# beer-asr/beer

Hardware: AMD Instinct MI355X
Metric: frames/sec per VB iteration (E+M) (higher is better)
Workload: dtype f32

## Files before the change

beer_amd/_hip.py:

```python

import ctypes
import os
import threading

import torch

_HERE = os.path.dirname(os.path.abspath(__file__))
LIB_PATH = os.environ.get('BEER_HIP_LIB') or os.path.join(_HERE, 'csrc', 'libbeer_hip.so')

F32, F64, I16 = 0, 1, 2
FULL, DIAG, ISO = 0, 1, 2
SEG = 8
MAX_HUBS = 4
COV_CODE = {'full': FULL, 'diagonal': DIAG, 'isotropic': ISO}
EINVAL = -100000


class HipUnavailable(RuntimeError):
    'Raised when the HIP extension or the GPU is missing (no CPU fallback).'


class HipError(RuntimeError):
    rc = None


class HipInvalid(HipError):
    rc = EINVAL


_lib = None


def lib():
    global _lib
    if _lib is None:
        if not os.path.exists(LIB_PATH):
            raise HipUnavailable(
                f'{LIB_PATH} is missing: build it with `python -m beer_amd.build` '
                '(beer_amd has no CPU fallback)')
        _lib = ctypes.CDLL(LIB_PATH)
        _declare(_lib)
        _options_from_env(_lib)
    return _lib


OPTIONS = {'ax_max_frames': (0, 'BEER_AX_MAXFRAMES'), 'accf_rounds': (1, 'BEER_ACCF_ROUNDS'),
           'accfi_waves': (2, 'BEER_ACCFI_WAVES'), 'lnfi': (3, 'BEER_LNFI'),
           'fb_log': (4, 'BEER_FB_LOG'), 'k1_lds': (5, 'BEER_K1_LDS')}


def _options_from_env(l):
    for name, (code, env) in OPTIONS.items():
        text = os.environ.get(env)
        if text is None:
            continue
        try:
            value = int(text)
        except ValueError:
            raise ValueError(f'{env}={text!r}: expected an integer') from None
        if l.beer_hip_set_option(code, value) != 0:
            raise ValueError(f'{env}={value}: outside the range of option {name!r} '
                             '(include/beer_hip.h)')


def set_option(name, value):
    code = OPTIONS[name][0]
    old = lib().beer_hip_get_option(code)
    if lib().beer_hip_set_option(code, int(value)) != 0:
        raise ValueError(f'option {name!r}: value {value} out of range')
    return old


def get_option(name):
    return lib().beer_hip_get_option(OPTIONS[name][0])


c_p, c_i, c_l, c_d = ctypes.c_void_p, ctypes.c_int, ctypes.c_int64, ctypes.c_double
c_z = ctypes.c_size_t


class Graph(ctypes.Structure):
    _fields_ = [('n_states', ctypes.c_int32), ('n_arcs', ctypes.c_int32),
                ('n_in_seg', ctypes.c_int32), ('n_out_seg', ctypes.c_int32),
                ('init', c_p), ('final', c_p),
                ('in_ptr', c_p), ('in_src', c_p), ('in_dst', c_p), ('in_w', c_p),
                ('in_seg', c_p), ('in_row_seg', c_p),
                ('out_ptr', c_p), ('out_dst', c_p), ('out_src', c_p), ('out_w', c_p),
                ('out_seg', c_p), ('out_row_seg', c_p), ('lowdeg', c_p)]


class GraphLowDeg(ctypes.Structure):
    _fields_ = [('n_arcs', ctypes.c_int32), ('n_hubs', ctypes.c_int32),
                ('in_ptr', c_p), ('in_src', c_p), ('in_w', c_p),
                ('out_ptr', c_p), ('out_dst', c_p), ('out_w', c_p),
                ('hub_src_id', c_p), ('hub_src_w', c_p), ('hub_dst_id', c_p),
                ('hub_dst_w', c_p), ('src_ptr', c_p), ('src_list', c_p),
                ('dst_ptr', c_p), ('dst_list', c_p)]


class Batch(ctypes.Structure):
    _fields_ = [('nutt', ctypes.c_int32), ('max_states', ctypes.c_int32),
                ('max_arcs', ctypes.c_int32), ('max_segs', ctypes.c_int32),
                ('all_lowdeg', ctypes.c_int32), ('n_graphs', ctypes.c_int32),
                ('frame_off', c_p), ('llh_off', c_p), ('graph_id', c_p),
                ('graphs', c_p), ('pdf_off', c_p), ('pdf_ids', c_p),
                ('max_degree', ctypes.c_int32), ('max_hubs', ctypes.c_int32),
                ('max_hub_members', ctypes.c_int32), ('reserved', ctypes.c_int32),
                ('order', c_p)]


class CatMap(ctypes.Structure):
    _fields_ = [('arc_cat', c_p), ('last_cat', c_p), ('arc_off', c_p), ('state_off', c_p)]


class Bigram(ctypes.Structure):
    _fields_ = [('n_states', ctypes.c_int32), ('n_phones', ctypes.c_int32),
                ('max_degree', ctypes.c_int32), ('reserved', ctypes.c_int32),
                ('init', c_p), ('final', c_p),
                ('in_ptr', c_p), ('in_src', c_p), ('in_w', c_p),
                ('out_ptr', c_p), ('out_dst', c_p), ('out_w', c_p),
                ('src', c_p), ('dst', c_p), ('block_w', c_p),
                ('src_slot', c_p), ('dst_slot', c_p), ('pdf_ids', c_p)]


FB_WAVE, FB_LOWDEG, FB_GENERAL, FB_GENERAL_BIG = 0x1000, 0x2000, 0x3000, 0x4000


def fb_family(route):
    return route & 0xF000


SAMPLE_ARCS_LDS, SAMPLE_QUAD = 0x100, 0x200


def sample_chunk(route):
    return route & 0xFF


def sample_waves(route):
    return (route >> 12) & 0xF


ESTEP_PLAIN, ESTEP_PACKED, ESTEP_IMAGE = 0, 1, 2
ARG_PC_LLH, ARG_LOG_NORM, ARG_RESPS, ARG_LLH_SUM, ARG_LABELS, ARG_SCALED, ARG_LOG_WEIGHTS = \
    1, 2, 4, 8, 16, 32, 64
ESTEP_GENERIC, ESTEP_EXACT_F32, ESTEP_EXACT_F64, ESTEP_LLHX, ESTEP_LNFI = \
    0x10000000, 0x20000000, 0x30000000, 0x40000000, 0x50000000
ESTEP_GENERIC_PASS1, ESTEP_GENERIC_FUSED, ESTEP_GENERIC_NORMALISE, ESTEP_GENERIC_LABELS = 1, 2, 3, 4
ESTEP_X_PACKED, ESTEP_X_LNO, ESTEP_X_IMG, ESTEP_X_BL = 0x100, 0x200, 0x400, 0x800
ESTEP_X_NARROW, ESTEP_X_LANE_MAJOR, ESTEP_X_PADDED, ESTEP_X_XT = 0x1000, 0x2000, 0x4000, 0x8000


def estep_family(route):
    return route & 0x70000000


def estep_route(entry, dtype_code_, cov, D, S, G, args, workspace_bytes):
    return lib().beer_estep_route(entry, dtype_code_, cov, D, S, G, args, workspace_bytes)


ACC_PLAIN, ACC_PACKED, ACC_FUSED = 0, 1, 2
ARG_STATE_RESPS, ARG_IMAGE = 128, 256
ACC_GENERIC, ACC_EXACT_F32, ACC_EXACT_F64, ACC_DIAG, ACC_ACCX, ACC_ACCF = \
    0x10000000, 0x20000000, 0x30000000, 0x40000000, 0x50000000, 0x60000000
ACC_SR = 0x100
ACC_D_PARTIAL = 0x200
ACC_X_SX, ACC_X_XT_REUSED = 0x200, 0x400
ACC_F_BLK, ACC_F_IMAGE = 0x200, 0x400


def accumulate_family(route):
    return route & 0x70000000


def accumulate_route(entry, dtype_code_, cov, T, D, S, G, args, workspace_bytes):
    return lib().beer_accumulate_route(entry, dtype_code_, cov, T, D, S, G, args, workspace_bytes)


DENSE_LLH, DENSE_BACKWARD, DENSE_ACCUMULATE = 0, 1, 2
DENSE_PLAIN, DENSE_GEMM3 = 0x10000000, 0x20000000
DENSE_T64x128, DENSE_T128x64, DENSE_T128x128 = 1, 2, 3
DENSE_AK, DENSE_BK = 0x10, 0x20


def dense_family(route):
    return route & 0x70000000


def dense_chain(route):
    return (route >> 8 & 0xFF) * 32


def dense_route(op, dtype_code_, T, Q, K):
    return lib().beer_dense_route(op, dtype_code_, T, Q, K)


SGRAD_GENERIC, SGRAD_FULL, SGRAD_DIAG, SGRAD_CHUNKED = 0x10000000, 0x20000000, 0x30000000, 0x40000000


def sgrad_family(route):
    return route & 0x70000000


def sgrad_form(route):
    return route & 0x0FFFFFFF


def frames_llh_backward_route(dtype_code_, cov, T, D, K, workspace_bytes):
    return lib().beer_frames_llh_backward_route(dtype_code_, cov, T, D, K, workspace_bytes)


BIGRAM_MAX_PHONES = 128
BIGRAM_MAX_STATES = 512


class FeaConf(ctypes.Structure):
    _fields_ = [('flen', ctypes.c_int32), ('fstep', ctypes.c_int32),
                ('fft_len', ctypes.c_int32), ('mode', ctypes.c_int32),
                ('nfilters', ctypes.c_int32), ('apply_log', ctypes.c_int32),
                ('n_dct', ctypes.c_int32), ('add_energy', ctypes.c_int32),
                ('preemph', ctypes.c_double), ('log_offset', ctypes.c_double),
                ('norm', ctypes.c_double),
                ('window', c_p), ('filters', c_p), ('filt_lo', c_p), ('filt_hi', c_p),
                ('dct', c_p), ('lifter', c_p)]


_four = [c_i, c_i, c_i, c_p, c_p, c_p, c_p, c_p, c_p]
_from = [c_i, c_i, c_i, c_p, c_p, c_p, c_p, c_p, c_p]
_dir = [c_i, c_i, c_i, c_p, c_p, c_p]
_gam = [c_i, c_i, c_p, c_p, c_p, c_p]
SIGNATURES = {
    'beer_hip_version': [],
    'beer_hip_device_count': [],
    'beer_hip_set_option': [c_i, c_i],
    'beer_hip_get_option': [c_i],
    'beer_mixtureset_packed_supported': [c_i, c_i, c_i, c_i],
    'beer_nw_expected_stats': _four, 'beer_nw_log_norm': _four, 'beer_nw_natural': _four,
    'beer_nw_from_natural': _from,
    'beer_nw_expected_stats_log_norm': [c_i, c_i, c_i, c_p, c_p, c_p, c_p, c_p, c_p, c_p],
    'beer_nw_update': [c_i, c_i, c_i, c_p, c_p, c_p, c_p, c_p, c_p, c_p, c_p, c_p],
    'beer_ng_expected_stats': _four, 'beer_ng_log_norm': _four, 'beer_ng_natural': _four,
    'beer_ng_from_natural': _from,
    'beer_ing_expected_stats': _four, 'beer_ing_log_norm': _four, 'beer_ing_natural': _four,
    'beer_ing_from_natural': _from,
    'beer_dirichlet_expected_stats': _dir, 'beer_dirichlet_log_norm': _dir,
    'beer_dirichlet_natural': _dir, 'beer_dirichlet_from_natural': _dir,
    'beer_dirichlet_log_weights': _dir,
    'beer_sb_transform_stats': [c_i, c_i, c_p, c_p, c_p, c_p],
    'beer_sb_log_weights': [c_i, c_i, c_p, c_p, c_p, c_p, c_p],
    'beer_sb_set_log_weights': [c_i, c_i, c_i, c_p, c_p, c_p, c_p],
    'beer_sb_set_transform_stats': [c_i, c_i, c_i, c_p, c_p, c_p, c_p],
    'beer_gamma_expected_stats': _gam, 'beer_gamma_log_norm': _gam,
    'beer_gamma_natural': _gam,
    'beer_gamma_from_natural': [c_i, c_i, c_p, c_p, c_p, c_p],
    'beer_kl_div': [c_i, c_i, c_i, c_p, c_p, c_p, c_p, c_p, c_p, c_p],
    'beer_natural_grad_step': [c_i, c_l, c_p, c_p, c_p, c_d, c_p, c_p],
    'beer_suffstats_expand': [c_i, c_i, c_l, c_i, c_p, c_p, c_p],
    'beer_mixtureset_estep': [c_i, c_i, c_l, c_i, c_i, c_i, c_p, c_p, c_p, c_p, c_d,
                              c_p, c_p, c_p, c_p, c_p, c_z, c_p],
    'beer_normal_accumulate': [c_i, c_i, c_l, c_i, c_i, c_i, c_p, c_p, c_p, c_p, c_p, c_z,
                               c_p],
    'beer_mixture_estep_packed': [c_i, c_l, c_i, c_i, c_p, c_p, c_p, c_p, c_p, c_p, c_p, c_z,
                                  c_p],
    'beer_normal_accumulate_packed': [c_i, c_l, c_i, c_i, c_p, c_p, c_p, c_p, c_z, c_p],
    'beer_mixtureset_estep_packed': [c_i, c_l, c_i, c_i, c_i, c_p, c_p, c_p, c_p, c_p, c_p, c_p,
                                     c_z, c_p],
    'beer_mixtureset_accumulate_packed': [c_i, c_l, c_i, c_i, c_i, c_p, c_p, c_p, c_p, c_p, c_z,
                                          c_p],
    'beer_unpack_resps': [c_l, c_i, c_p, c_p, c_p],
    'beer_mixtureset_accumulate_fused': [c_i, c_l, c_i, c_i, c_i, c_p, c_p, c_p, c_p, c_p, c_p,
                                         c_p, c_p, c_z, c_p],
    'beer_frame_image': [c_i, c_l, c_i, c_p, c_p, c_z, c_p],
    'beer_mixtureset_lognorm_image': [c_i, c_l, c_i, c_i, c_i, c_p, c_p, c_p, c_p, c_p, c_p, c_p,
                                      c_z, c_p],
    'beer_estep_route': [c_i, c_i, c_i, c_i, c_i, c_i, ctypes.c_uint, c_z],
    'beer_accumulate_route': [c_i, c_i, c_i, c_l, c_i, c_i, c_i, ctypes.c_uint, c_z],
    'beer_dense_route': [c_i, c_i, c_l, c_i, c_i],
    'beer_frames_llh_backward_route': [c_i, c_i, c_l, c_i, c_i, c_z],
    'beer_pack_resps': [c_l, c_i, c_i, c_i, c_p, c_p, c_p, c_p, c_p],
    'beer_weights_from_acc': [c_i, c_i, c_i, c_p, c_p, c_p],
    'beer_tied_lognorm': [c_i, c_l, c_i, c_i, c_p, c_p, c_p, c_p, c_p, c_p],
    'beer_tied_accumulate': [c_i, c_l, c_i, c_i, c_p, c_p, c_p, c_p, c_p, c_p, c_p, c_p],
    'beer_hmm_gather': [c_i, c_p, c_i, c_p, c_d, c_p, c_p],
    'beer_hmm_forward_backward': [c_i, c_p, c_p, c_p, c_p, c_p, c_p, c_p, c_p, c_p, c_p],
    'beer_hmm_posteriors_fused': [c_i, c_p, c_i, c_p, c_d, c_p, c_p, c_p, c_i, c_p, c_p, c_p,
                                  c_p, c_p],
    'beer_hmm_posteriors_fused_counts': [c_i, c_p, c_i, c_p, c_d, c_p, c_p, c_p, c_i, c_p, c_p,
                                         c_p, c_p, c_p, c_p, c_p],
    'beer_hmm_forward_backward_counts': [c_i, c_p, c_p, c_p, c_p, c_p, c_p, c_p, c_p, c_p, c_p,
                                         c_p],
    'beer_hmm_last_frame_sum': [c_i, c_p, c_p, c_p, c_p],
    'beer_hmm_refresh_weights': [c_i, c_l, c_p, c_p, c_p, c_p, c_p],
    'beer_hmm_posteriors_fused_cat': [c_i, c_p, c_i, c_p, c_d, c_p, c_p, c_p, c_i, c_p, c_p, c_p,
                                      c_p, c_p, c_p],
    'beer_hmm_forward_backward_cat': [c_i, c_p, c_p, c_p, c_p, c_p, c_p, c_p, c_p, c_p, c_p],
    'beer_hmm_path_counts_cat': [c_p, c_p, c_p, c_p, c_p],
    'beer_hmm_fb_log_count': [c_p, c_p, c_p, c_p],
    'beer_hmm_fb_route': [c_i, c_p, c_i, c_i],
    'beer_hmm_posteriors_bigram': [c_i, c_p, ctypes.c_int32, c_l, c_p, c_p, c_i, c_p, c_d, c_p,
                                   c_p, c_p, c_i, c_p, c_p],
    'beer_hmm_bigram_route': [c_i, c_p, ctypes.c_int32, ctypes.c_int32],
    'beer_hmm_viterbi': [c_i, c_p, c_p, c_p, c_p, c_i, c_p],
    'beer_hmm_sample_paths': [c_i, c_p, c_p, c_p, ctypes.c_int32, c_p, c_p, c_i, c_p],
    'beer_hmm_sample_route': [c_i, c_p, ctypes.c_int32],
    'beer_hmm_trans_posteriors': [c_i, c_l, c_i, c_p, c_p, c_p, c_p, c_p, c_p],
    'beer_hmm_path_posteriors': [c_i, c_p, c_p, c_p, c_p, c_p, c_p],
    'beer_hmm_scatter': [c_i, c_p, c_i, c_p, c_p, c_d, c_p, c_p, c_p, c_p],
    'beer_segment_sum': [c_i, ctypes.c_int32, c_p, c_p, c_p, c_p],
    'beer_dense_llh': [c_i, c_l, c_i, c_i, c_p, c_p, c_d, c_p, c_p],
    'beer_dense_llh_backward': [c_i, c_l, c_i, c_i, c_p, c_p, c_p, c_p, c_p],
    'beer_dense_accumulate': [c_i, c_l, c_i, c_i, c_i, c_p, c_p, c_p, c_p, c_p],
    'beer_rowdot': [c_i, c_l, c_i, c_p, c_p, c_p, c_p],
    'beer_softmax_groups': [c_i, c_l, c_i, c_i, c_p, c_p, c_p, c_p, c_p],
    'beer_features_signal_mean': [c_i, ctypes.c_int32, c_p, c_p, c_p, c_p],
    'beer_features_extract': [c_i, ctypes.c_int32, c_p, c_p, c_l, c_p, c_p, c_p, c_p,
                              ctypes.c_int32, c_p],
    'beer_features_deltas': [ctypes.c_int32, c_p, c_l, ctypes.c_int32, ctypes.c_int32,
                             ctypes.c_int32, c_p, c_p, c_p],
    'beer_features_cmn': [ctypes.c_int32, c_p, ctypes.c_int32, ctypes.c_int32, c_p, c_p],
    'beer_copy_pinned': [c_p, c_p, c_z, c_p],
    'beer_clock_probe': [c_p, c_i, c_p],
    'beer_suffstats_mean': [c_i, c_i, c_l, c_i, c_i, c_p, c_p, c_p],
    'beer_suffstats_backward': [c_i, c_i, c_l, c_i, c_i, c_p, c_p, c_p, c_p],
    'beer_frames_llh_backward': [c_i, c_i, c_l, c_i, c_i, c_p, c_p, c_p, c_p, c_p, c_p, c_z, c_p],
}


c_pp = ctypes.POINTER(ctypes.c_void_p)
HOST_SIGNATURES = {
    'beer_graph_compile': [ctypes.c_int32, c_p, c_l, c_p, c_p, c_p, ctypes.c_int32,
                           ctypes.c_int32, c_pp],
    'beer_aligraphs_compile': [ctypes.c_int32, c_p, c_p, c_p, c_p, c_p, c_p, c_p, c_p, c_l,
                               c_p, c_p, c_pp],
    'beer_graphset_from_csr': [c_l, c_p, c_p, c_p, c_p, c_p, c_p, c_p, c_p, c_pp],
    'beer_graphset_free': [c_p],
    'beer_graphset_sizes': [c_p, c_p, c_p, c_p],
    'beer_graphset_export': [c_p, c_p, c_p, c_p, c_p, c_p, c_p],
    'beer_graphset_image_bytes': [c_p, c_i, c_p],
    'beer_graphset_image': [c_p, c_i, c_p, ctypes.c_uint64, c_p],
}

SIZE_QUERIES = {
    'beer_estep_workspace_bytes': [c_i, c_i, c_i, c_i, c_i],
    'beer_accumulate_workspace_bytes': [c_i, c_i, c_i, c_i, c_i],
    'beer_accumulate_frames_workspace_bytes': [c_i, c_i, c_l, c_i, c_i, c_i],
    'beer_packed_resps_bytes': [c_l, c_i, c_i],
    'beer_accumulate_fused_workspace_bytes': [c_i, c_i, c_i, c_i],
    'beer_frame_image_bytes': [c_i, c_l, c_i],
    'beer_accumulate_packed_workspace_bytes': [c_i, c_l, c_i, c_i],
    'beer_mixtureset_accumulate_packed_workspace_bytes': [c_i, c_l, c_i, c_i, c_i],
    'beer_hmm_fb_scratch_doubles': [c_i, c_p, c_i],
    'beer_frames_llh_backward_workspace_bytes': [c_i, c_i, c_l, c_i, c_i],
}


def _declare(l):
    for name, args in SIGNATURES.items():
        fn = getattr(l, name)
        fn.argtypes = args
        fn.restype = c_i
    for name, args in HOST_SIGNATURES.items():
        fn = getattr(l, name)
        fn.argtypes = args
        fn.restype = c_i
    for name, args in SIZE_QUERIES.items():
        fn = getattr(l, name)
        fn.argtypes = args
        fn.restype = c_z


def dtype_code(dtype, exact=False):
    if dtype == torch.float32:
        return F32 | EXACT if exact else F32
    if dtype == torch.float64:
        return F64
    raise TypeError(f'beer_amd kernels take float32 or float64 tensors, got {dtype}')


def require_device():
    if not torch.cuda.is_available():
        raise HipUnavailable('beer_amd needs an AMD GPU (gfx950); there is no CPU fallback')
    lib()
    return torch.device('cuda', torch.cuda.current_device())


def on_device(t, dtype=None):
    dev = require_device()
    if t.device.type != 'cuda':
        t = t.to(dev)
    if dtype is not None and t.dtype != dtype:
        t = t.to(dtype)
    return t.contiguous()


def ptr(t):
    return None if t is None else ctypes.c_void_p(t.data_ptr())


def stream_id():
    return torch.cuda.current_stream().cuda_stream


def stream():
    return ctypes.c_void_p(stream_id())


def call(name, *args):
    rc = getattr(lib(), name)(*args, stream())
    if rc == EINVAL:
        raise HipInvalid(f'{name} failed: invalid argument')
    if rc != 0:
        err = HipError(f'{name} failed: hipError {-rc}')
        err.rc = rc
        raise err


EXACT = 0x10
F32_MODES = ('exact', 'bf16x3')
_f32_mode = ['exact' if os.environ.get('BEER_F32_MODE') in ('exact', 'f32') else 'bf16x3']


def set_f32_mode(mode):
    if mode not in F32_MODES:
        raise ValueError(f'f32 mode {mode!r}: expected one of {F32_MODES}')
    _f32_mode[0] = mode


def get_f32_mode():
    return _f32_mode[0]


FAST_MIN_FRAMES = 16384
MAX_DIM_F32 = 96
MAX_DIM_FAST = 128


def f32_fast_ok(X):
    return X.dtype == torch.float32 and get_f32_mode() == 'bf16x3' and \
        X.shape[0] >= FAST_MIN_FRAMES and X.shape[1] <= MAX_DIM_FAST


class exact_f32:

    def __enter__(self):
        self.old = get_f32_mode()
        set_f32_mode('exact')

    def __exit__(self, *exc):
        set_f32_mode(self.old)


def call_host(name, *args):
    rc = getattr(lib(), name)(*args)
    if rc != 0:
        raise HipInvalid(f'{name} failed: invalid argument')


_workspaces = {}


def scratch(key, nbytes, device):
    if nbytes == 0:
        return None, 0
    key = (key, device, stream_id())
    buf = _workspaces.get(key)
    if buf is None or buf.numel() < nbytes:
        buf = _workspaces[key] = torch.empty(nbytes, dtype=torch.uint8, device=device)
    return buf, nbytes


def workspace(query, dtype, cov, D, S, G, device):
    return scratch((query, dtype, cov, D, S, G),
                   getattr(lib(), query)(dtype_code(dtype), cov, D, S, G), device)


def frames_workspace(dtype, exact, cov, T, D, S, G, device):
    return scratch(('frames', dtype, cov, D, S, G), lib().beer_accumulate_frames_workspace_bytes(
        dtype_code(dtype, exact), cov, T, D, S, G), device)


def packed_workspace(cov, T, D, K, device, sets=None):
    if sets is None:
        nbytes = lib().beer_accumulate_packed_workspace_bytes(cov, T, D, K)
    else:
        nbytes = lib().beer_mixtureset_accumulate_packed_workspace_bytes(cov, T, D, *sets)
    return scratch(('packed', cov, D, K), nbytes, device)


_staging = threading.local()


def _staging_buffer(nbytes):
    ring = _staging.__dict__.setdefault('ring', [])
    if not ring:
        for _ in range(4):
            ring.append([torch.empty(1 << 20, dtype=torch.uint8, pin_memory=True),
                         torch.cuda.Event()])
    nxt = _staging.__dict__.get('next', 0)
    slot = ring[nxt % len(ring)]
    _staging.next = nxt + 1
    slot[1].synchronize()
    if slot[0].numel() < nbytes:
        slot[0] = torch.empty(max(nbytes, 2 * slot[0].numel()), dtype=torch.uint8,
                              pin_memory=True)
# ... 38 lines not shown
```

beer_amd/csrc/estep.hip:

```cpp

#include "common.h"
#include "estep_mfma.h"

using namespace beer;

namespace {

constexpr int kFrameTile = 64;
constexpr int kLlhThreads = 256;
constexpr int kCompChunk = 64;

template <typename T, int COV>
__global__ __launch_bounds__(kLlhThreads) void llh_kernel(
    int64_t nframes, int D, int K, const T* __restrict__ X, const T* __restrict__ expT,
    const T* __restrict__ logw, double stat_scale, T* __restrict__ pc_llh,
    T* __restrict__ w_out, int fuse_G, T* __restrict__ log_norm,
    double* __restrict__ llh_sum) {
    extern __shared__ __attribute__((aligned(16))) char smem[];
    const int ldx = D + 1;
    T* xs = reinterpret_cast<T*>(smem);
    T* outs = xs + kFrameTile * ldx;
    const int ldo = kCompChunk + 1;
    const int Q = stats_dim(COV, D);
    const int64_t t0 = (int64_t)blockIdx.x * kFrameTile;
// ... 275 lines not shown
                         ws_bytes >= beer_mfma::estep_workspace_bytes(elem, cov, D, S, G);
    const bool split_ws = elem == 4 && !exact &&
                          ws_bytes >= beer_mfma::estepx_workspace_bytes(cov, D, S, G) &&
                          beer_mfma::estepx_workspace_bytes(cov, D, S, G) > 0;
    const bool aligned_x = split_ws && beer_mfma::supported_llh_x(D, S, G);
    const bool padded = split_ws && !comp_resps && beer_mfma::supported_llh_split(D, S, G);
    p.use_x = aligned_x || padded;
    const bool mfma_ok = !labels && !pc_llh && unscaled && ws && (aligned || p.use_x) &&
                         (log_norm || comp_resps || llh_sum);
    p.use_x = mfma_ok && p.use_x;
    p.exact_mfma = mfma_ok && !p.use_x;
    if (p.need_norm && !comp_resps && !mfma_ok && !(G == 1 && log_norm)) return p;
    if (labels && !(pc_llh || comp_resps)) return p;
    p.pc_in_resps = labels && !pc_llh;
    p.fuse = !mfma_ok && p.need_norm && !labels && (kCompChunk % G == 0) && (comp_resps || G == 1);
    p.rc = BEER_OK;
    return p;
}

template <typename T>
int estep_launch(int cov, int64_t nframes, int D, int S, int G, const void* X, const void* expT,
                 const void* logw, const int64_t* labels, double stat_scale, void* pc_llh,
                 void* log_norm, void* comp_resps, double* llh_sum, void* ws, size_t ws_bytes,
                 void* stream, bool exact) {
    BEER_REQUIRE(nframes >= 0 && X && expT);
    const EstepPlan p = estep_plan(sizeof(T), exact, cov, D, S, G, pc_llh, log_norm, comp_resps,
                                   llh_sum, labels, stat_scale == 1.0, ws, ws_bytes);
    if (p.rc != BEER_OK || nframes == 0) return p.rc;
    hipStream_t s = as_stream(stream);
    if (p.use_x)
        return beer_mfma::estep_bf16x3(cov, nframes, D, S, G, (const float*)X, (const float*)expT,
                                       (const float*)logw, (float*)comp_resps, (float*)log_norm,
                                       llh_sum, ws, ws_bytes, s);
    if (p.exact_mfma)
        return sizeof(T) == 4
                   ? beer_mfma::estep_f32(cov, nframes, D, S, G, (const float*)X,
                                          (const float*)expT, (const float*)logw,
                                          (float*)comp_resps, (float*)log_norm, llh_sum, ws,
                                          ws_bytes, s)
                   : beer_mfma::estep_f64(cov, nframes, D, S, G, (const double*)X,
                                          (const double*)expT, (const double*)logw,
                                          (double*)comp_resps, (double*)log_norm, llh_sum, ws,
                                          ws_bytes, s);
    const int K = S * G;
    void* pc = p.pc_in_resps ? comp_resps : pc_llh;
    static_assert(BEER_FULL == 0 && BEER_DIAG == 1 && BEER_ISO == 2, "pass1 is indexed by cov");
    constexpr decltype(&llh_launch<T, BEER_FULL>) pass1[] = {
        llh_launch<T, BEER_FULL>, llh_launch<T, BEER_DIAG>, llh_launch<T, BEER_ISO>};
    const int rc = pass1[cov](nframes, D, K, X, expT, logw, stat_scale, pc,
                              p.need_norm ? comp_resps : nullptr, p.fuse ? G : 0,
                              p.fuse ? log_norm : nullptr, p.fuse ? llh_sum : nullptr, s);
    if (rc != BEER_OK) return rc;
    if (labels) {
        hipLaunchKernelGGL(labels_kernel<T>, dim3((unsigned)((nframes + 255) / 256)), dim3(256), 0,
                           s, nframes, K, labels, (const T*)pc, (T*)comp_resps, (T*)log_norm,
                           llh_sum);
        BEER_LAUNCH_CHECK();
    } else if (p.need_norm && !p.fuse) {
        const int64_t n = nframes * S;
        hipLaunchKernelGGL(normalise_kernel<T>, dim3((unsigned)((n + 255) / 256)), dim3(256), 0, s,
                           nframes, S, G, (T*)comp_resps, (T*)log_norm, true, llh_sum);
        BEER_LAUNCH_CHECK();
    }
    return BEER_OK;
}

template <typename T, int COV>
int acc_launch(int64_t nframes, int D, int S, int G, const void* X, const void* cr,
               const void* sr, double* acc, hipStream_t s) {
    const int K = S * G, Q = stats_dim(COV, D);
    const int gx = (Q + kAccThreads - 1) / kAccThreads, gy = (K + kAccKB - 1) / kAccKB;
    int64_t gz = (256LL * 4 + (int64_t)gx * gy - 1) / ((int64_t)gx * gy);
    const int64_t min_frames = nframes >= 65536 ? 512 : kAccTile;
    const int64_t max_z = (nframes + min_frames - 1) / min_frames;
    if (gz > max_z) gz = max_z;
    if (gz < 1) gz = 1;
    if (gz > 65535) gz = 65535;
    const beer_mfma::FrameSplit z = beer_mfma::frame_split(nframes, gz, kAccTile);
    const size_t lds = ((size_t)kAccTile * D + (size_t)kAccTile * kAccKB) * sizeof(T);
    hipLaunchKernelGGL((accumulate_kernel<T, COV>), dim3(gx, gy, (unsigned)z.gz), dim3(kAccThreads),
                       lds, s, nframes, D, S, G, (const T*)X, (const T*)cr, (const T*)sr, z.fpb, acc);
    BEER_LAUNCH_CHECK();
    return BEER_OK;
}

struct AccPlan {
    int rc;
    bool diag;
    bool exact_mfma;
};

AccPlan accumulate_plan(size_t elem, bool exact, int cov, int64_t nframes, int D, int S, int G,
                        bool cr, bool sr, bool ws, size_t ws_bytes) {
    AccPlan p = {};
    p.rc = BEER_EINVAL;
    if (!(nframes >= 0 && D >= 1 && S >= 1 && G >= 1 && cov >= 0 && cov <= 2)) return p;
    p.rc = BEER_OK;
    p.diag = elem == 4 && !exact && cr && !sr &&
             beer_mfma::supported_acc_diag(cov, nframes, D, S * G);
    p.exact_mfma = !p.diag && cr && ws && beer_mfma::supported_acc(D, S * G, elem) &&
                   ws_bytes >= beer_mfma::acc_workspace_bytes(cov, D, S * G, elem);
    return p;
}

template <typename T>
int accumulate_launch(int cov, int64_t nframes, int D, int S, int G, const void* X,
                      const void* cr, const void* sr, double* acc, void* ws, size_t ws_bytes,
                      void* stream, bool exact) {
    const AccPlan p = accumulate_plan(sizeof(T), exact, cov, nframes, D, S, G, cr, sr, ws, ws_bytes);
    BEER_REQUIRE(p.rc == BEER_OK && X && acc);
    if (nframes == 0) return BEER_OK;
    hipStream_t s = as_stream(stream);
    if (p.diag)
        return beer_mfma::acc_diag_bf16x3(cov, nframes, D, S * G, (const float*)X,
                                          (const float*)cr, acc, ws, ws_bytes, s);
    if (p.exact_mfma)
        return sizeof(T) == 4
                   ? beer_mfma::acc_f32(cov, nframes, D, S, G, (const float*)X, (const float*)cr,
                                        (const float*)sr, acc, ws, ws_bytes, s)
                   : beer_mfma::acc_f64(cov, nframes, D, S, G, (const double*)X,
                                        (const double*)cr, (const double*)sr, acc, ws, ws_bytes,
                                        s);
    constexpr decltype(&acc_launch<T, BEER_FULL>) generic[] = {
        acc_launch<T, BEER_FULL>, acc_launch<T, BEER_DIAG>, acc_launch<T, BEER_ISO>};
    return generic[cov](nframes, D, S, G, X, cr, sr, acc, s);
}

template <typename T>
int segment_sum_launch(int32_t nutt, const int64_t* frame_off, const void* v, double* out,
                       void* stream) {
    BEER_REQUIRE(nutt >= 0);
    if (nutt == 0) return BEER_OK;
    hipLaunchKernelGGL(segment_sum_kernel<T>, dim3(nutt), dim3(256), 0, as_stream(stream),
                       frame_off, (const T*)v, out);
    BEER_LAUNCH_CHECK();
    return BEER_OK;
}

int estepx_refusal(int entry, bool set, int cov, int D, int S, int G, unsigned args,
                   size_t ws_bytes) {
    const bool packed = entry == BEER_ESTEP_PACKED, resps = args & BEER_ARG_RESPS;
    BEER_REQUIRE(D >= 1 && S >= 1 && G >= 1 && cov >= 0 && cov <= 2);
    BEER_REQUIRE(!(args & (BEER_ARG_PC_LLH | BEER_ARG_LABELS | BEER_ARG_SCALED)));
    if (packed)
        BEER_REQUIRE(resps && (set ? beer_mixtureset_packed_supported(cov, D, S, G)
                                   : S == 1 && (args & BEER_ARG_LOG_WEIGHTS)));
    else
        BEER_REQUIRE((args & BEER_ARG_LOG_NORM) && !resps);
    return beer_mfma::llhx_form(cov, D, S, G, packed, packed, !packed, ws_bytes).rc;
}

int estepx_entry(int entry, bool set, int cov, int64_t T, int D, int S, int G, const float* X,
                 const float* exp_stats, const float* logw, const void* image, float* log_norm,
                 void* resps, double* llh_sum, void* ws, size_t ws_bytes, void* stream) {
    const unsigned args = (log_norm ? BEER_ARG_LOG_NORM : 0u) | (resps ? BEER_ARG_RESPS : 0u) |
                          (llh_sum ? BEER_ARG_LLH_SUM : 0u) | (logw ? BEER_ARG_LOG_WEIGHTS : 0u);
    const int rc = estepx_refusal(entry, set, cov, D, S, G, args, ws ? ws_bytes : 0);
    if (rc != BEER_OK || T == 0) return rc;
    return beer_mfma::estep_bf16x3(cov, T, D, S, G, X, exp_stats, logw, (float*)resps, log_norm,
                                   llh_sum, ws, ws_bytes, as_stream(stream),
                                   entry == BEER_ESTEP_PACKED, image);
}

int accx_refusal(bool set, int cov, int64_t T, int D, int S, int G, size_t ws_bytes) {
    BEER_REQUIRE(T >= 0 && D >= 1 && S >= 1 && G >= 1 && cov >= 0 && cov <= 2);
    BEER_REQUIRE(!set || beer_mixtureset_packed_supported(cov, D, S, G));
    BEER_REQUIRE(beer_mfma::accx_form(cov, D, S * G, S, G, set).rc == BEER_OK);
    const size_t need = beer_mfma::accx_layout(cov, T, D, S * G, S, G, set).bytes;
    BEER_REQUIRE(need > 0 && ws_bytes >= need);
    return BEER_OK;
}
int accf_refusal(int cov, int64_t T, int D, int S, int G, size_t ws_bytes) {
    BEER_REQUIRE(T >= 0 && D >= 1 && S >= 1 && G >= 1 && cov >= 0 && cov <= 2);
    BEER_REQUIRE(beer_mfma::accf_form(cov, D, S, G, false).rc == BEER_OK);
    const size_t need = beer_mfma::accf_layout(cov, D, S, G).bytes;
    BEER_REQUIRE(need > 0 && ws_bytes >= need);
    return BEER_OK;
}

}

extern "C" {

int beer_mixtureset_estep(int dtype, int cov, int64_t T, int D, int S, int G, const void* X,
                          const void* exp_stats, const void* log_weights,
                          const int64_t* labels, double stat_scale, void* pc_llh,
                          void* log_norm, void* comp_resps, double* llh_sum, void* workspace,
                          size_t workspace_bytes, void* stream) {
    const bool exact = (dtype & BEER_EXACT) != 0;
    BEER_DISPATCH(dtype & ~BEER_EXACT, estep_launch, cov, T, D, S, G, X, exp_stats, log_weights,
                  labels, stat_scale, pc_llh, log_norm, comp_resps, llh_sum, workspace,
                  workspace_bytes, stream, exact);
}

int beer_estep_route(int entry, int dtype, int cov, int D, int S, int G, unsigned args,
                     size_t workspace_bytes) {
    const bool exact = (dtype & BEER_EXACT) != 0;
    dtype &= ~BEER_EXACT;
    BEER_REQUIRE(dtype == BEER_F32 || dtype == BEER_F64);
    const bool resps = args & BEER_ARG_RESPS, labels = args & BEER_ARG_LABELS;
    bool packed = false;
    if (entry == BEER_ESTEP_PLAIN) {
        const EstepPlan p = estep_plan(dtype == BEER_F64 ? 8 : 4, exact, cov, D, S, G,
                                       args & BEER_ARG_PC_LLH, args & BEER_ARG_LOG_NORM, resps,
                                       args & BEER_ARG_LLH_SUM, labels, !(args & BEER_ARG_SCALED),
                                       workspace_bytes > 0, workspace_bytes);
        if (p.rc != BEER_OK) return p.rc;
        if (p.exact_mfma) {
            const beer_mfma::LlhForm f = beer_mfma::llh_form(S, G);
            return (dtype == BEER_F64 ? BEER_ESTEP_EXACT_F64 : BEER_ESTEP_EXACT_F32) | f.NT |
                   f.GQ << 5 | f.jw << 8 | (f.nchunks > 0xfff ? 0xfff : f.nchunks) << 16;
        }
        if (!p.use_x)
            return BEER_ESTEP_GENERIC | (labels ? BEER_ESTEP_GENERIC_LABELS
                                         : !p.need_norm ? BEER_ESTEP_GENERIC_PASS1
                                         : p.fuse ? BEER_ESTEP_GENERIC_FUSED
                                                  : BEER_ESTEP_GENERIC_NORMALISE);
    } else if (entry == BEER_ESTEP_PACKED || entry == BEER_ESTEP_IMAGE) {
        BEER_REQUIRE(dtype == BEER_F32 && !exact);
        BEER_REQUIRE(estepx_refusal(entry, S != 1, cov, D, S, G, args, workspace_bytes) == BEER_OK);
        packed = entry == BEER_ESTEP_PACKED;
    } else {
        return BEER_EINVAL;
    }
    const beer_mfma::LlhxForm x = beer_mfma::llhx_form(cov, D, S, G, resps, packed,
                                                       entry == BEER_ESTEP_IMAGE, workspace_bytes);
    if (x.rc != BEER_OK) return x.rc;
    const int nchunks = (x.nchunks > 0xfff ? 0xfff : x.nchunks) << 16;
    if (x.lnfi) return BEER_ESTEP_LNFI | x.NT | x.nku << 5 | x.lnfi_g << 8 | nchunks;
    return BEER_ESTEP_LLHX | x.NT | x.GQ << 5 | (x.packed ? BEER_ESTEP_X_PACKED : 0) |
           (x.lno ? BEER_ESTEP_X_LNO : 0) | (x.img ? BEER_ESTEP_X_IMG : 0) |
           (x.bl ? BEER_ESTEP_X_BL : 0) | (x.narrow ? BEER_ESTEP_X_NARROW : 0) |
           (x.lane_major ? BEER_ESTEP_X_LANE_MAJOR : 0) | (x.Gp != G ? BEER_ESTEP_X_PADDED : 0) |
           (x.xt ? BEER_ESTEP_X_XT : 0) | nchunks;
}

size_t beer_estep_workspace_bytes(int dtype, int cov, int D, int S, int G) {
    if (cov < 0 || cov > 2) return 0;
    dtype &= ~BEER_EXACT;
    const size_t exact = beer_mfma::estep_workspace_bytes(dtype == BEER_F64 ? 8 : 4, cov, D, S, G);
    if (dtype == BEER_F64) return exact;
    const size_t split = beer_mfma::estepx_workspace_bytes(cov, D, S, G);
    return exact > split ? exact : split;
}

size_t beer_accumulate_workspace_bytes(int dtype, int cov, int D, int S, int G) {
    if (cov < 0 || cov > 2) return 0;
    return beer_mfma::acc_workspace_bytes(cov, D, S * G, (dtype & ~BEER_EXACT) == BEER_F64 ? 8 : 4);
}

size_t beer_accumulate_frames_workspace_bytes(int dtype, int cov, int64_t T, int D, int S, int G) {
    const size_t base = beer_accumulate_workspace_bytes(dtype, cov, D, S, G);
    if (dtype != BEER_F32 || T < 0 || S < 1 || G < 1) return base;
    const size_t rows = beer_mfma::acc_diag_workspace_bytes(cov, T, D, S * G);
    return rows > base ? rows : base;
}

int beer_normal_accumulate(int dtype, int cov, int64_t T, int D, int S, int G, const void* X,
                           const void* comp_resps, const void* state_resps, double* acc,
                           void* workspace, size_t workspace_bytes, void* stream) {
    const bool exact = (dtype & BEER_EXACT) != 0;
    BEER_DISPATCH(dtype & ~BEER_EXACT, accumulate_launch, cov, T, D, S, G, X, comp_resps,
                  state_resps, acc, workspace, workspace_bytes, stream, exact);
}

int beer_accumulate_route(int entry, int dtype, int cov, int64_t T, int D, int S, int G,
                          unsigned args, size_t workspace_bytes) {
    const bool exact = (dtype & BEER_EXACT) != 0;
    dtype &= ~BEER_EXACT;
    BEER_REQUIRE(dtype == BEER_F32 || dtype == BEER_F64);
    const bool sets = args & BEER_ARG_STATE_RESPS;
    if (entry == BEER_ACC_PLAIN) {
        const size_t elem = dtype == BEER_F64 ? 8 : 4;
        const AccPlan p = accumulate_plan(elem, exact, cov, T, D, S, G, args & BEER_ARG_RESPS, sets,
                                          workspace_bytes > 0, workspace_bytes);
        if (p.rc != BEER_OK) return p.rc;
        if (p.diag) {
            const beer_mfma::AccdForm f = beer_mfma::accd_form(cov, T, D, S * G, workspace_bytes);
            return f.rc != BEER_OK ? f.rc
                                   : BEER_ACC_DIAG | f.NJ2 | f.NC << 4 |
                                         (f.partial ? BEER_ACC_D_PARTIAL : 0);
        }
        if (p.exact_mfma) {
            const beer_mfma::AccForm f = beer_mfma::acc_form(elem, cov, D, S * G, sets);
            return f.rc != BEER_OK ? f.rc
                                   : (elem == 8 ? BEER_ACC_EXACT_F64 : BEER_ACC_EXACT_F32) | f.NQ |
                                         (f.has_sr ? BEER_ACC_SR : 0);
        }
        return BEER_ACC_GENERIC;
    }
    BEER_REQUIRE(dtype == BEER_F32 && !exact);
    if (entry == BEER_ACC_PACKED) {
        BEER_REQUIRE(args & BEER_ARG_RESPS);
        BEER_REQUIRE(accx_refusal(sets, cov, T, D, S, G, workspace_bytes) == BEER_OK);
        const beer_mfma::AccxForm f = beer_mfma::accx_form(cov, D, S * G, S, G, sets);
        return BEER_ACC_ACCX | f.NQ | (f.sr ? BEER_ACC_SR : 0) | (f.sx ? BEER_ACC_X_SX : 0) |
               (f.xt_reused ? BEER_ACC_X_XT_REUSED : 0);
    }
    if (entry == BEER_ACC_FUSED) {
        BEER_REQUIRE(accf_refusal(cov, T, D, S, G, workspace_bytes) == BEER_OK);
        const beer_mfma::AccfForm f = beer_mfma::accf_form(cov, D, S, G, args & BEER_ARG_IMAGE);
        if (f.use_image)
            return BEER_ACC_ACCF | BEER_ACC_F_IMAGE | f.NKU << 4 | f.ns_img << 16 | f.waves << 21;
        return BEER_ACC_ACCF | f.NQT | (f.blk ? BEER_ACC_F_BLK : 0) | f.waves << 21;
    }
    return BEER_EINVAL;
}

int beer_mixture_estep_packed(int cov, int64_t T, int D, int K, const float* X,
                              const float* exp_stats, const float* log_weights, float* log_norm,
                              void* packed_resps, double* llh_sum, void* workspace,
                              size_t workspace_bytes, void* stream) {
    BEER_REQUIRE(T >= 0 && X && exp_stats);
    return estepx_entry(BEER_ESTEP_PACKED, false, cov, T, D, 1, K, X, exp_stats, log_weights, nullptr,
                        log_norm, packed_resps, llh_sum, workspace, workspace_bytes, stream);
}

int beer_normal_accumulate_packed(int cov, int64_t T, int D, int K, const float* X,
                                  const void* packed_resps, double* acc, void* workspace,
                                  size_t workspace_bytes, void* stream) {
    BEER_REQUIRE(X && packed_resps && acc && workspace);
    BEER_REQUIRE(accx_refusal(false, cov, T, D, 1, K, workspace_bytes) == BEER_OK);
    if (T == 0) return BEER_OK;
    return beer_mfma::acc_bf16x3_packed(cov, T, D, K, X, packed_resps, acc, workspace,
                                        workspace_bytes, as_stream(stream));
}

int beer_mixtureset_packed_supported(int cov, int D, int S, int G) {
    return cov >= 0 && cov <= 2 && D >= 1 && D <= beer_mfma::kMaxDimX && S >= 1 && G >= 1 &&
           beer_mfma::supported_llh_packed_sets(cov, D, S, G) &&
           beer_mfma::supported_acc_sets(cov, D, S, G);
}

size_t beer_mixtureset_accumulate_packed_workspace_bytes(int cov, int64_t T, int D, int S, int G) {
    if (T < 0 || !beer_mixtureset_packed_supported(cov, D, S, G)) return 0;
    return beer_mfma::accxs_workspace_bytes(cov, T, D, S, G);
}

int beer_mixtureset_estep_packed(int cov, int64_t T, int D, int S, int G, const float* X,
                                 const float* exp_stats, const float* log_weights,
                                 float* log_norm, void* packed_resps, double* llh_sum,
                                 void* workspace, size_t workspace_bytes, void* stream) {
    BEER_REQUIRE(T >= 0 && X && exp_stats);
    return estepx_entry(BEER_ESTEP_PACKED, true, cov, T, D, S, G, X, exp_stats, log_weights, nullptr,
                        log_norm, packed_resps, llh_sum, workspace, workspace_bytes, stream);
}

int beer_mixtureset_accumulate_packed(int cov, int64_t T, int D, int S, int G, const float* X,
                                      const void* packed_resps, const float* state_resps,
                                      double* acc, void* workspace, size_t workspace_bytes,
                                      void* stream) {
    BEER_REQUIRE(X && packed_resps && state_resps && acc && workspace);
    BEER_REQUIRE(accx_refusal(true, cov, T, D, S, G, workspace_bytes) == BEER_OK);
    if (T == 0) return BEER_OK;
    return beer_mfma::acc_bf16x3_packed(cov, T, D, S * G, X, packed_resps, acc, workspace,
                                        workspace_bytes, as_stream(stream), S, G, state_resps);
}

size_t beer_accumulate_fused_workspace_bytes(int cov, int D, int S, int G) {
    if (cov < 0 || cov > 2 || D < 1 || S < 1 || G < 1) return 0;
    return beer_mfma::accf_workspace_bytes(cov, D, S, G);
}

int beer_mixtureset_lognorm_image(int cov, int64_t T, int D, int S, int G, const float* X,
                                  const float* exp_stats, const float* log_weights,
                                  const void* frame_image, float* log_norm, double* llh_sum,
                                  void* workspace, size_t workspace_bytes, void* stream) {
    BEER_REQUIRE(T >= 0 && frame_image && (T == 0 || (X && exp_stats)));
    return estepx_entry(BEER_ESTEP_IMAGE, true, cov, T, D, S, G, X, exp_stats, log_weights,
                        frame_image, log_norm, nullptr, llh_sum, workspace, workspace_bytes, stream);
}

size_t beer_frame_image_bytes(int cov, int64_t T, int D) {
    if (cov < 0 || cov > 2 || T < 0 || D < 1) return 0;
    return beer_mfma::frame_image_bytes(cov, T, D);
}

int beer_frame_image(int cov, int64_t T, int D, const float* X, void* image, size_t image_bytes,
                     void* stream) {
    BEER_REQUIRE(cov >= 0 && cov <= 2 && T >= 0 && D >= 1);
    const size_t need = beer_mfma::frame_image_bytes(cov, T, D);
    BEER_REQUIRE(need > 0 && image && image_bytes >= need && (T == 0 || X));
    return beer_mfma::frame_image(cov, T, D, X, image, as_stream(stream));
}

int beer_mixtureset_accumulate_fused(int cov, int64_t T, int D, int S, int G, const float* X,
                                     const float* exp_stats, const float* log_weights,
                                     const float* log_norm, const float* state_resps,
                                     const void* frame_image, double* acc, void* workspace,
                                     size_t workspace_bytes, void* stream) {
    BEER_REQUIRE(accf_refusal(cov, T, D, S, G, workspace ? workspace_bytes : 0) == BEER_OK);
    if (T == 0) return BEER_OK;
    BEER_REQUIRE(X && exp_stats && log_norm && acc);
    return beer_mfma::acc_fused_bf16x3(cov, T, D, S, G, X, exp_stats, log_weights, log_norm,
                                       state_resps, frame_image, acc, workspace, workspace_bytes,
                                       as_stream(stream));
}

size_t beer_packed_resps_bytes(int64_t T, int D, int K) {
    return T < 0 || D < 1 || D > beer_mfma::kMaxDimX || K < 1 ? 0 : beer_mfma::packed_resps_bytes(T, D, K);
}

size_t beer_accumulate_packed_workspace_bytes(int cov, int64_t T, int D, int K) {
    if (cov < 0 || cov > 2 || T < 0 || D < 1 || K < 1) return 0;
    return beer_mfma::accx_workspace_bytes(cov, T, D, K);
}

int beer_pack_resps(int64_t T, int D, int S, int G, const float* X, const float* comp_resps,
                    const float* state_resps, void* packed_resps, void* stream) {
    BEER_REQUIRE(T >= 0 && D >= 1 && D <= beer_mfma::kMaxDimX && S >= 1 && G >= 1 && (S * G) % 4 == 0);
    BEER_REQUIRE(T == 0 || (X && comp_resps && packed_resps));
    return beer_mfma::pack_resps(T, D, S, G, X, comp_resps, state_resps, packed_resps,
                                 as_stream(stream));
}

int beer_unpack_resps(int64_t T, int K, const void* packed_resps, float* resps, void* stream) {
    BEER_REQUIRE(T >= 0 && K >= 1 && (T == 0 || (packed_resps && resps)));
    return beer_mfma::unpack_resps(T, K, packed_resps, resps, as_stream(stream));
}

int beer_weights_from_acc(int S, int G, int Q, const double* acc, double* out, void* stream) {
    BEER_REQUIRE(S >= 0 && G >= 1 && Q >= 3 && acc && out);
    if (S == 0) return BEER_OK;
    hipLaunchKernelGGL(weights_from_acc_kernel, dim3(S), dim3(64), 0,
                       as_stream(stream), S, G, Q, acc, out);
    BEER_LAUNCH_CHECK();
    return BEER_OK;
}

int beer_segment_sum(int dtype, int32_t nutt, const int64_t* frame_off, const void* v,
                     double* out, void* stream) {
    BEER_DISPATCH(dtype, segment_sum_launch, nutt, frame_off, v, out, stream);
}

}
```

beer_amd/csrc/estep_bf16.hip:

```cpp

#include <cstdlib>
#include <type_traits>
#include <utility>

#include "estep_mfma.h"
#include "estep_tiles.h"

namespace beer_mfma {

namespace {

typedef __bf16 bf8 __attribute__((ext_vector_type(8)));
typedef unsigned int u4 __attribute__((ext_vector_type(4)));
typedef float f32x2 __attribute__((ext_vector_type(2)));

template <int V> using ic = std::integral_constant<int, V>;
template <int... I, typename F>
__device__ __forceinline__ void static_for_impl(std::integer_sequence<int, I...>, F&& f) {
    (f(ic<I>{}), ...);
}
template <int N, typename F>
__device__ __forceinline__ void static_for(F&& f) {
    static_for_impl(std::make_integer_sequence<int, N>{}, static_cast<F&&>(f));
}

constexpr int NP = kPackedPieces;
constexpr int kProdA[6] = {0, 0, 1, 0, 1, 2};
constexpr int kProdB[6] = {0, 1, 0, 2, 1, 0};

__device__ __forceinline__ bf8 as_bf8(const u4& w) { return __builtin_bit_cast(bf8, w); }
__device__ __forceinline__ f32x4 mfma_bf16(const u4& a, const u4& b, const f32x4& c) {
    return __builtin_amdgcn_mfma_f32_16x16x32_bf16(as_bf8(a), as_bf8(b), c, 0, 0, 0);
}
template <bool FIRST>
__device__ __forceinline__ void mfma_bf16_pinned(f32x4& acc, const u4& a, const u4& b) {
    if (FIRST)
        asm volatile("s_nop 1\n\tv_mfma_f32_16x16x32_bf16 %0, %1, %2, %0" : "+a"(acc) : "v"(a), "v"(b));
    else
        asm volatile("v_mfma_f32_16x16x32_bf16 %0, %1, %2, %0" : "+a"(acc) : "v"(a), "v"(b));
}
__device__ __forceinline__ void mfma_bf16_pinned_v(f32x4& acc, const u4& a, const u4& b) {
    asm volatile("v_mfma_f32_16x16x32_bf16 %0, %1, %2, %0" : "+v"(acc) : "v"(a), "v"(b));
}
__device__ __forceinline__ void mfma_drain() {
    asm volatile("s_nop 15\n\ts_nop 15" ::: "memory");
    __builtin_amdgcn_sched_barrier(0);
}

__host__ __device__ inline size_t frame_image_tile_u4(int nk_used, int nqt) {
    return (size_t)(nk_used * NP * 2 + nqt * NP) * 64;
}
__host__ __device__ constexpr int img_nqt(int nk_used) { return nk_used <= 3 ? 5 : 6; }
constexpr int kImgMaxNK = 4;
__host__ __device__ inline int stat_slab(int j) { return j + j / 7; }
__host__ __device__ inline int nk16_of(int cov, int D) {
    return ((nslabx_of(cov, D) + 7) / 8 + 1) / 2 * 2;
}
__host__ __device__ inline int ld16_of(int D) {
    const int ld = 4 * d4_of(D) + 8;
    return (ld / 4) % 2 ? ld : ld + 4;
}
constexpr float kConstEps = 5.9604644775390625e-8f;
constexpr int kBlockU4 = NP * 64;

__device__ inline double entry_value(int cov, int D, int K, int k, int slab, int e,
                                     const float* __restrict__ row, bool* is_const) {
    const int D4 = d4_of(D), Dp = 4 * D4, nslab = nslabx_of(cov, D);
    *is_const = false;
    if (slab >= nslab) return 0.0;
    if (band_layout(cov, D)) {
        const int nb = band_nslab(D);
        if (slab == nslab - 1) {
            *is_const = true;
            return 0.0;
        }
        if (k >= K) return 0.0;
        if (slab >= nb) {
            const int b = 4 * (slab - nb) + e;
            return b < D ? (double)row[b] : 0.0;
        }
        int a, b;
        if (!band_pair(D, slab, e, &a, &b)) return 0.0;
        return b == a ? -0.5 * (double)row[D + a * D + a]
                      : -0.5 * ((double)row[D + a * D + b] + (double)row[D + b * D + a]);
    }
    const int t = slab_entry(cov, D, slab);
    const int a = t & 0xff, b = ((t >> 8) & 0xff) + e, sq = t >> 16;
    if (a == Dp && b - e == Dp) {
        *is_const = true;
        return 0.0;
    }
    if (k >= K) return 0.0;
    if (sq) return b < D ? -0.5 * (double)row[cov == BEER_ISO ? D : D + b] : 0.0;
    if (a < D) {
        if (b >= D || b < a) return 0.0;
        return b == a ? -0.5 * (double)row[D + a * D + a]
                      : -0.5 * ((double)row[D + a * D + b] + (double)row[D + b * D + a]);
    }
    return b < D ? (double)row[b] : 0.0;
}

__global__ __launch_bounds__(256) void const_max_kernel(int cov, int D, int K,
                                                        const float* __restrict__ E,
                                                        const float* __restrict__ logw,
                                                        float* __restrict__ c0) {
    __shared__ double red[8];
    const int Q = stats_dim(cov, D);
    double m = -1.0e300;
    for (int k = threadIdx.x; k < K; k += blockDim.x) {
        const double v = const_total(cov, D, E + (size_t)k * Q, logw ? (double)logw[k] : 0.0);
        if (v == v && v > m && v < 1.0e300) m = v;
    }
    m = block_max(m, red);
    if (threadIdx.x == 0) c0[0] = m > -1.0e300 ? (float)m : 0.f;
}

__global__ __launch_bounds__(256) void packx_kernel(int cov, int D, int K, int NT,
                                                    const float* __restrict__ E,
                                                    const float* __restrict__ logw,
                                                    unsigned short* __restrict__ P,
                                                    int* __restrict__ tab, int G, int Gp,
                                                    const float* __restrict__ c0, int lane_major) {
    extern __shared__ __attribute__((aligned(16))) char pack_lds[];
    const int nk = nk16_of(cov, D), nent = nk * 32;
    const int slot = blockIdx.x;
    const int k = slot % Gp < G ? (slot / Gp) * G + slot % Gp : K;
    const int chunk = slot / (NT * 16), kk = slot % (NT * 16);
    const int c = lane_major ? kk % NT : 4 * (kk / 64) + (kk % 4);
    const int i = lane_major ? kk / NT : (kk % 64) / 4;
    if (slot == 0)
        for (int s = threadIdx.x; s < (nk + 1) * 8; s += blockDim.x) tab[s] = slabx_entry(cov, D, s);
    const int Qs = stats_dim(cov, D);
    float* rowl = reinterpret_cast<float*>(pack_lds);
    if (k < K)
        for (int q = threadIdx.x; q < Qs; q += blockDim.x) rowl[q] = E[(size_t)k * Qs + q];
    __syncthreads();
    unsigned short* base = P + ((size_t)chunk * nk * NT) * (NP * 512);
    auto put = [&](int q, float v) {
        const int s = q / 32, g = (q % 32) / 8, j = q % 8;
        unsigned short* dst = base + ((size_t)s * NT + c) * (NP * 512) + (g * 16 + i) * 8 + j;
        unsigned short p[3];
        split3_scalar(v, p);
        dst[0] = p[0];
        dst[512] = p[1];
        dst[1024] = p[2];
    };
    const int nslab = nslabx_of(cov, D);
    for (int q = threadIdx.x; q < nent; q += blockDim.x) {
        bool is_const;
        const double v = entry_value(cov, D, K, k, q / 4, q % 4, rowl, &is_const);
        if (!is_const) {
            put(q, (float)v);
        } else if (q % 4 == 0) {
            const bool last = q / 4 == nslab - 1;
            const double want = k < K ? const_share(cov, D, q / 4, rowl, logw ? (double)logw[k] : 0.0) -
                                            (last ? (double)c0[0] : 0.0)
                                      : (last ? kPadLogit : 0.0);
            const float hi = (float)want;
            const double rem = (want - (double)hi) * (1.0 / (double)kConstEps);
            put(q, hi);
            put(q + 1, (rem == rem && fabs(rem) < 1.0e30) ? (float)rem : 0.f);
            put(q + 2, 0.f);
            put(q + 3, 0.f);
        }
    }
}

inline int xcd_chunk_group(int ny, size_t chunk_bytes) {
    int cg = (int)((size_t)(2 << 20) / (chunk_bytes ? chunk_bytes : 1));
    return cg < 1 ? 1 : (cg > ny ? ny : cg);
}
inline unsigned xcd_grid(int64_t nx, int ny, int cg) {
    return (unsigned)((nx + 7) / 8 * 8 * cg * ((ny + cg - 1) / cg));
}
__device__ inline bool xcd_block(int64_t nx, int ny, int cg, int64_t& bx, int& by) {
    const unsigned per_group = (unsigned)((nx + 7) / 8 * 8 * cg);
    const unsigned grp = blockIdx.x / per_group, rem = blockIdx.x - grp * per_group;
    const unsigned xcd = rem & 7, slot = rem >> 3;
    by = (int)(grp * cg + slot % (unsigned)cg);
    bx = (int64_t)(slot / (unsigned)cg) * 8 + xcd;
    return bx < nx && by < ny;
}

template <int FW>
__device__ __forceinline__ void stage_rows(const float* __restrict__ X, int64_t fb,
                                           int64_t nframes, int D, int LD, int lane,
                                           float* __restrict__ xw) {
    const int Dp = 4 * d4_of(D);
    if ((D & 3) == 0) {
        constexpr int LPR = 64 / FW, NPC = kMaxDimX / 4 / LPR;
        const int C4 = D >> 2, r = lane & (FW - 1), h = lane / FW;
        const int64_t f = fb + r;
        const bool valid = f < nframes;
        const f32x4* src = reinterpret_cast<const f32x4*>(X) + (valid ? f : nframes - 1) * C4;
        f32x4 xv[NPC];
#pragma unroll
        for (int it = 0; it < NPC; ++it) {
            const int pc = h + LPR * it;
            xv[it] = src[pc < C4 ? pc : C4 - 1];
        }
#pragma unroll
        for (int it = 0; it < NPC; ++it) {
            const int pc = h + LPR * it;
            if (pc < C4)
                *reinterpret_cast<f32x4*>(xw + r * LD + 4 * pc) =
                    valid ? xv[it] : f32x4{0.f, 0.f, 0.f, 0.f};
        }
        for (int idx = lane; idx < FW * ((LD - D) / 4); idx += 64) {
            const int rr = idx / ((LD - D) / 4), hh = idx - rr * ((LD - D) / 4);
            *reinterpret_cast<f32x4*>(xw + rr * LD + D + 4 * hh) =
                f32x4{hh == 0 ? 1.f : 0.f, hh == 0 ? kConstEps : 0.f, 0.f, 0.f};
        }
    } else {
        for (int idx = lane; idx < FW * LD; idx += 64) {
            const int r = idx / LD, c = idx - r * LD;
            const int64_t f = fb + r;
            float v = 0.f;
            if (c < D) { if (f < nframes) v = X[f * D + c]; }
            else if (c == Dp) v = 1.f;
            else if (c == Dp + 1) v = kConstEps;
            xw[idx] = v;
        }
    }
}

__device__ __forceinline__ int k1_slab_word(int t, int Dp) {
    int w = t & 0xff;
#pragma unroll
    for (int e = 0; e < 4; ++e) w |= band_col(t, e, Dp) << (6 + 6 * e);
    return w;
}

template <int NT, int MT, int GQ, bool PACKED, bool SQ, bool LNO, bool IMG = false, bool BL = false>
__global__ __launch_bounds__(kThreads, 2) void llhx_kernel(
    int64_t nframes, int D, int K, int S, int G, int gl, int jw, int nk,
    const float* __restrict__ X, const u4* __restrict__ Pall, const int* __restrict__ tab,
    float* __restrict__ resps, float* __restrict__ log_norm, double* __restrict__ llh_sum,
    float* __restrict__ xt_out, int xt_floats, int nku, int cg, const float* __restrict__ c0,
    const u4* __restrict__ img = nullptr) {
    static_assert(MT * NT <= 32, "128 accumulators: two waves per SIMD (launch bounds)");
    static_assert(!IMG || (MT == 2 && !PACKED && LNO), "the image holds 32-frame tiles");
    static_assert(!BL || (NT == 16 && MT == 2 && !IMG && !SQ), "half k-steps of 8 tiles, band slabs");
    extern __shared__ __attribute__((aligned(16))) char smem[];
    const int LD = ld16_of(D);
    const int Dp = 4 * d4_of(D);
    const int tid = threadIdx.x, lane = tid & 63;
    const int wave = __builtin_amdgcn_readfirstlane(tid >> 6);
    const int i = lane & 15, g = lane >> 4;
    constexpr int FW = 16 * MT, NW = kThreads / 64;
    float* xw = reinterpret_cast<float*>(smem) + wave * (FW * LD);
    int* tabs = reinterpret_cast<int*>(reinterpret_cast<float*>(smem) + NW * FW * LD);
    constexpr int kHalfBytes = 8 * kBlockU4 * 16;
    char* ring = smem + (((size_t)NW * FW * LD * sizeof(float) + (size_t)(nk + 1) * 8 * sizeof(int)
                          + 1023) & ~(size_t)1023);
    int64_t bx = blockIdx.x;
    int by = 0;
    {
        const int nch = (K + 16 * NT - 1) / (16 * NT);
        constexpr int FBK = FW * NW;
        if (nch > 1 && !xcd_block((nframes + FBK - 1) / FBK, nch, cg, bx, by)) return;
    }
    const int64_t fb = (bx * NW + wave) * FW;
    for (int idx = tid; idx < (nk + 1) * 8; idx += kThreads)
        tabs[idx] = BL ? k1_slab_word(tab[idx], Dp) : tab[idx];
    if (!IMG) stage_rows<FW>(X, fb, nframes, D, LD, lane, xw);
    __syncthreads();
    if (IMG && fb >= nframes) return;
    {
        static_assert(64 % FW == 0, "whole waves per 64-frame tile");
        if (xt_out && by == 0 && fb < (nframes + 63) / 64 * 64) {
            float* img = xt_out + (fb / 64) * (size_t)xt_floats;
            const int c0 = (int)(fb % 64);
            const int ncol4 = FW / 4 + (c0 + FW == 64 ? 1 : 0);
            for (int e4 = lane; e4 < (D + 2) * ncol4; e4 += 64) {
                const int row = e4 / ncol4, c = 4 * (e4 - row * ncol4);
                f32x4 v = {0.f, 0.f, 0.f, 0.f};
                if (row < D) {
#pragma unroll
                    for (int j = 0; j < 4; ++j) v[j] = c + j < FW ? xw[(c + j) * LD + row] : 0.f;
                } else if (row == D) {
                    v = f32x4{1.f, 1.f, 1.f, 1.f};
                }
                __builtin_nontemporal_store(v, reinterpret_cast<f32x4*>(img + row * 68 + c0 + c));
            }
        }
    }

    f32x4 acc[MT][NT];
#pragma unroll
    for (int m = 0; m < MT; ++m)
#pragma unroll
        for (int c = 0; c < NT; ++c) acc[m][c] = f32x4{0, 0, 0, 0};

    const float* xrow[MT];
#pragma unroll
    for (int m = 0; m < MT; ++m) xrow[m] = xw + (m * 16 + i) * LD;

    const int kbase = by * (16 * NT);
    const u4* Pl = Pall + (size_t)by * nk * NT * kBlockU4 + lane;
    const int* tl = tabs + 2 * g;

    struct AFrag { u4 w[NP][MT]; };
    auto make_half = [&](int s, int m, int h, AFrag& f) {
        const int t = tl[8 * s + h];
        f32x4 p;
        if constexpr (SQ) {
            const int a = t & 0xff, j = (t >> 8) & 0xff;
            const bool sq = (t >> 16) != 0;
            const f32x4 bb = *reinterpret_cast<const f32x4*>(xrow[m] + j);
// ... 1505 lines not shown
                                                    packed_tiles_bytes(nframes, K)));
    BEER_LAUNCH_CHECK();
    return BEER_OK;
}

int unpack_resps(int64_t nframes, int K, const void* packed, float* resps, hipStream_t s) {
    const int64_t n = nframes * K;
    if (n == 0) return BEER_OK;
    hipLaunchKernelGGL(unpack_resps_kernel, dim3((unsigned)((n + 255) / 256)), dim3(256), 0, s,
                       nframes, K, reinterpret_cast<const unsigned*>(packed), resps);
    BEER_LAUNCH_CHECK();
    return BEER_OK;
}

size_t estepx_workspace_bytes(int cov, int D, int S, int G) {
    if (!supported_llh_padded(D, S, G)) return 0;
    if (S > 1) G = group_pad(G);
    const int K = S * G, NT = ntx_for(S, K), nchunks = nchunksx_for(S, K);
    return ptab_layout(nchunks, nk16_of(cov, D), NT).c0 + 256;
}

bool supported_frame_image(int cov, int D);

LlhxForm llhx_form(int cov, int D, int S, int G, bool resps, bool packed, bool image,
                   size_t ws_bytes) {
    LlhxForm f = {};
    f.rc = BEER_EINVAL;
    if (packed && S != 1 && !supported_llh_packed_sets(cov, D, S, G)) return f;
    if (!supported_llh_padded(D, S, G) || ws_bytes < estepx_workspace_bytes(cov, D, S, G))
        return f;
    const int Greal = G;
    if (S > 1) G = group_pad(G);
    if (G != Greal && resps) return f;
    f.Gp = G;
    f.packed = packed;
    const int K = S * G;
    f.narrow = S > 1 && Greal == 1 && K <= 128 && !packed && !image;
    f.lnfi8 = image && !f.narrow && S > 1 && !resps && !packed && cov != BEER_FULL &&
              (nslab_of(cov, D) + 7) / 8 == 4 && (G == 4 || G == 8) &&
              beer::option(BEER_OPT_LNFI);
    f.NT = f.narrow ? (K <= 64 ? 4 : 8) : (f.lnfi8 ? 8 : ntx_for(S, K));
    f.nchunks = f.lnfi8 ? (K + 127) / 128 : nchunksx_for(S, K);
    if (image && (S == 1 || packed || resps || G < 4 || cov == BEER_FULL ||
                  !supported_frame_image(cov, D)))
        return f;
    f.rc = BEER_OK;
    f.lane_major = S > 1 && !resps && !packed &&
                   ((f.NT == 16 && (G == 4 || G == 8 || G == 16)) || f.lnfi8);
    const bool k1_lds = cov == BEER_FULL && k1_lds_fits(D, nk16_of(cov, D)) &&
                        beer::option(BEER_OPT_K1_LDS);
    if (S == 1) {
        f.gl = 16;
        f.jw = 4;
        f.GQ = f.NT == 4 ? 1 : (f.NT == 8 ? 2 : 4);
        f.xt = packed && f.NT == 16;
        f.bl = f.xt && k1_lds;
        return f;
    }
    f.jw = G < 4 ? G : 4;
    f.gl = f.lane_major ? 0 : (G < 4 ? 1 : (G < 64 ? G / 4 : 16));
    const int gq = G <= 64 ? 1 : G / 64;
    f.GQ = gq == 1 ? 1 : (gq == 2 ? 2 : 4);
    if (f.narrow) {
        f.GQ = 1;
        return f;
    }
    if (packed) {
        f.GQ = gq == 1 ? 1 : 2;
        f.bl = k1_lds;
        return f;
    }
    const int nku = (nslab_of(cov, D) + 7) / 8;
    if (image && f.lane_major && (nku <= 3 || f.lnfi8) && beer::option(BEER_OPT_LNFI)) {
        f.lnfi = true;
        f.nku = f.lnfi8 ? 4 : (nku == 1 ? 1 : (nku == 2 ? 2 : 3));
        f.lnfi_g = G == 4 ? 4 : (G == 8 ? 8 : 16);
        return f;
    }
    f.img = image;
    f.lno = image || (!resps && f.jw == 4);
    return f;
}

namespace {

int64_t lnfi_frames_per_workgroup(int64_t nframes, int nchunks) {
    int64_t best_fpb = 256, best_cost = -1;
    for (int64_t fpb = 256; fpb <= 8192; fpb += 256) {
        const int64_t wgs = (nframes + fpb - 1) / fpb * nchunks;
        const int64_t cost = (wgs + 255) / 256 * (fpb + 128);
        if (best_cost < 0 || cost < best_cost) { best_cost = cost; best_fpb = fpb; }
    }
    return best_fpb;
}

template <int NKU, int G, int NT>
int launch_lnfi(const LlhxArgs& a) {
    const int64_t fpb = lnfi_frames_per_workgroup(a.nframes, a.nchunks);
    const size_t lds = (size_t)NKU * NT * kBlockU4 * 16;
    const dim3 grid(xcd_grid((a.nframes + fpb - 1) / fpb, a.nchunks, a.nchunks));
    (void)hipFuncSetAttribute(reinterpret_cast<const void*>(lnfi_kernel<NKU, G, NT>),
                              hipFuncAttributeMaxDynamicSharedMemorySize, beer::kMaxDynLds);
    hipLaunchKernelGGL((lnfi_kernel<NKU, G, NT>), grid, dim3(512), lds, a.s, a.nframes, a.K, a.S,
                       a.nk, reinterpret_cast<const u4*>(a.img), reinterpret_cast<const u4*>(a.P),
                       a.log_norm, a.llh_sum, fpb, a.c0);
    BEER_LAUNCH_CHECK();
    return BEER_OK;
}

struct LlhxRow {
    int NT, GQ, nku;
    bool packed, lno, img, bl;
    int (*full)(const LlhxArgs&);
    int (*sq)(const LlhxArgs&);
};
template <int NT, int GQ, bool PACKED, bool LNO>
constexpr LlhxRow llhx_row() {
    return {NT, GQ, 0, PACKED, LNO, false, false, launch_llhx<NT, 2, GQ, PACKED, false, LNO>,
            launch_llhx<NT, 2, GQ, PACKED, true, LNO>};
}
template <int GQ>
constexpr LlhxRow bl_row() {
    return {16, GQ, 0, true, false, false, true,
            launch_llhx<16, 2, GQ, true, false, false, false, true>, nullptr};
}
template <int GQ>
constexpr LlhxRow img_row() {
    return {16, GQ, 0, false, true, true, false, nullptr,
            launch_llhx<16, 2, GQ, false, true, true, true>};
}
template <int NKU, int G, int NT>
constexpr LlhxRow lnfi_row() {
    return {NT, G, NKU, false, false, false, false, nullptr, launch_lnfi<NKU, G, NT>};
}
const LlhxRow kLlhxRows[] = {
    llhx_row<4, 1, true, false>(), llhx_row<8, 2, true, false>(), bl_row<4>(),
    llhx_row<16, 4, true, false>(),
    llhx_row<4, 1, false, false>(), llhx_row<8, 2, false, false>(), llhx_row<16, 4, false, false>(),
    llhx_row<8, 1, false, false>(),
    bl_row<1>(), bl_row<2>(), llhx_row<16, 1, true, false>(), llhx_row<16, 2, true, false>(),
    lnfi_row<4, 4, 8>(), lnfi_row<4, 8, 8>(),
    lnfi_row<1, 4, 16>(), lnfi_row<1, 8, 16>(), lnfi_row<1, 16, 16>(),
    lnfi_row<2, 4, 16>(), lnfi_row<2, 8, 16>(), lnfi_row<2, 16, 16>(),
    lnfi_row<3, 4, 16>(), lnfi_row<3, 8, 16>(), lnfi_row<3, 16, 16>(),
    img_row<1>(), img_row<2>(), img_row<4>(),
    llhx_row<16, 1, false, true>(), llhx_row<16, 2, false, true>(), llhx_row<16, 4, false, true>(),
    llhx_row<16, 1, false, false>(), llhx_row<16, 2, false, false>(),
};

}

int estep_bf16x3(int cov, int64_t nframes, int D, int S, int G, const float* X, const float* expT,
                 const float* logw, float* resps, float* log_norm, double* llh_sum, void* ws,
                 size_t ws_bytes, hipStream_t s, bool packed, const void* image) {
    const LlhxForm f = llhx_form(cov, D, S, G, resps != nullptr, packed, image != nullptr, ws_bytes);
    if (f.rc != BEER_OK) return f.rc;
    const int Kreal = S * G, nk = nk16_of(cov, D);
    LlhxArgs a = {};
    a.nframes = nframes, a.D = D, a.K = S * f.Gp, a.S = S, a.G = f.Gp;
    a.gl = f.gl, a.jw = f.jw, a.nchunks = f.nchunks, a.nk = nk;
    a.nku = (nslabx_of(cov, D) + 7) / 8;
    a.X = X, a.resps = resps, a.log_norm = log_norm, a.llh_sum = llh_sum, a.img = image, a.s = s;
    const PtabLayout l = ptab_layout(f.nchunks, nk, f.NT);
    int* tab = reinterpret_cast<int*>(reinterpret_cast<char*>(ws) + l.tab);
    float* c0 = reinterpret_cast<float*>(reinterpret_cast<char*>(ws) + l.c0);
    a.P = ws, a.tab = tab, a.c0 = c0;
    if (f.xt) {
        a.xt_out = reinterpret_cast<float*>(reinterpret_cast<char*>(resps) +
                                            packed_tiles_bytes(nframes, a.K));
        a.xt_floats = xt_pieces(D) * (kPiece / 4);
    }
    hipLaunchKernelGGL(const_max_kernel, dim3(1), dim3(256), 0, s, cov, D, Kreal, expT, logw, c0);
    hipLaunchKernelGGL(packx_kernel, dim3(f.nchunks * f.NT * 16), dim3(256),
                       (size_t)stats_dim(cov, D) * sizeof(float), s, cov, D, Kreal, f.NT, expT, logw,
                       reinterpret_cast<unsigned short*>(ws), tab, G, f.Gp, c0,
                       f.lane_major ? 1 : 0);
    BEER_LAUNCH_CHECK();
    const int nku = f.lnfi ? f.nku : 0, gq = f.lnfi ? f.lnfi_g : f.GQ;
    for (const LlhxRow& r : kLlhxRows)
        if (r.NT == f.NT && r.GQ == gq && r.nku == nku && r.packed == f.packed && r.lno == f.lno &&
            r.img == f.img && r.bl == f.bl) {
            const auto launch = cov == BEER_FULL ? r.full : r.sq;
            return launch ? launch(a) : BEER_EINVAL;
        }
    return BEER_EINVAL;
}


bool supported_acc_sets(int cov, int D, int S, int G) {
    return S >= 1 && G >= 8 && G <= 128 && (G & (G - 1)) == 0 && supported_acc_x(D, S * G);
}
inline int acc_sets_spad(int S, int G) {
    return (S * G + kPackedComps - 1) / kPackedComps * (kPackedComps / G);
}

AccxLayout accx_layout(int cov, int64_t nframes, int D, int K, int S, int G, bool sets) {
    AccxLayout l = {};
    if (!supported_acc_x(D, K) || (sets && !supported_acc_sets(cov, D, S, G))) return l;
    const int nslab = nslabx_of(cov, D);
    const int64_t tiles = (nframes + kAxFT - 1) / kAxFT;
    l.tab = up256((size_t)K * nslab * 4 * sizeof(double));
    l.Xt = l.tab + up256((size_t)nslab * sizeof(int)) + 1024;
    l.bytes = l.Xt + (size_t)tiles * xt_pieces(D) * kPiece;
    if (sets) {
        l.Gt = up256(l.bytes);
        l.bytes = l.Gt + (size_t)tiles * acc_sets_spad(S, G) * kAxFT * sizeof(float) + 1024;
    }
    return l;
}
size_t accx_workspace_bytes(int cov, int64_t nframes, int D, int K) {
    return accx_layout(cov, nframes, D, K, 1, K, false).bytes;
}
size_t accxs_workspace_bytes(int cov, int64_t nframes, int D, int S, int G) {
    return accx_layout(cov, nframes, D, S * G, S, G, true).bytes;
}

AccxForm accx_form(int cov, int D, int K, int S, int G, bool sets) {
    AccxForm f = {};
    f.rc = BEER_EINVAL;
    if (!supported_acc_x(D, K)) return f;
    if (sets && (S * G != K || !supported_acc_sets(cov, D, S, G))) return f;
    f.sr = sets;
    if (sets)
        while ((1 << f.lgG) < G) ++f.lgG;
    f.nslab = nslabx_of(cov, D);
    f.NX = xt_pieces(D);
    const int ntiles = (f.nslab * 4 + 15) / 16;
    f.NQ = accx_nq(ntiles);
    f.gx = (ntiles + f.NQ * kAxWaves - 1) / (f.NQ * kAxWaves);
    f.gy = (K + 16 * kAxMC - 1) / (16 * kAxMC);
    f.xt_reused = packed_has_xt(K) && !sets;
    const size_t rbuf = 2 * (size_t)NP * kPackedPlaneWords * 4 + (sets ? 2 * 4096 : 0);
    f.lds = 2 * (size_t)f.NX * kPiece + rbuf;
    f.sx = f.lds > (size_t)beer::kMaxDynLds;
    if (f.sx) f.lds = (size_t)f.NX * kPiece + rbuf;
    f.band = band_layout(cov, D);
    f.rc = BEER_OK;
    return f;
}

namespace {

struct AccxArgs {
    int64_t nframes, fpb;
    int D, K, nslab, NX, gx, gy, gz, lgG, sx, band;
    const float* Xt;
    const unsigned* R;
    const int* tab;
    double* Sp;
    const float* Gt;
    dim3 grid;
    size_t lds;
    hipStream_t s;
};

template <bool SR, int NQ>
int launch_accx(const AccxArgs& a) {
    (void)hipFuncSetAttribute(reinterpret_cast<const void*>(accx_kernel<SR, NQ>),
                              hipFuncAttributeMaxDynamicSharedMemorySize, beer::kMaxDynLds);
    hipLaunchKernelGGL((accx_kernel<SR, NQ>), a.grid, dim3(64 * kAxWaves), a.lds, a.s, a.nframes,
                       a.D, a.K, a.nslab, a.NX, a.Xt, a.R, a.tab, a.fpb, a.Sp, a.gx, a.gy, a.gz,
                       a.Gt, a.lgG, a.sx, a.band);
    BEER_LAUNCH_CHECK();
    return BEER_OK;
}
constexpr struct { bool sr; int NQ; int (*launch)(const AccxArgs&); } kAccxRows[] = {
    {true, 6, launch_accx<true, 6>},   {true, 7, launch_accx<true, 7>},
    {true, 8, launch_accx<true, 8>},   {false, 6, launch_accx<false, 6>},
    {false, 7, launch_accx<false, 7>}, {false, 8, launch_accx<false, 8>}};

int unpackx(int cov, int D, int K, const double* Sp, double* acc, hipStream_t s) {
    const int64_t total = (int64_t)K * stats_dim(cov, D);
    hipLaunchKernelGGL(unpackx_kernel, dim3((unsigned)((total + 255) / 256)), dim3(256), 0, s, cov,
                       D, K, Sp, acc);
    BEER_LAUNCH_CHECK();
    return BEER_OK;
}

}

int acc_bf16x3_packed(int cov, int64_t nframes, int D, int K, const float* X, const void* Rimg,
                      double* acc, void* ws, size_t ws_bytes, hipStream_t s, int S, int G,
                      const float* SR) {
    const AccxForm f = accx_form(cov, D, K, S, G, SR != nullptr);
    const AccxLayout l = accx_layout(cov, nframes, D, K, S, G, SR != nullptr);
    if (f.rc != BEER_OK || ws_bytes < l.bytes) return BEER_EINVAL;
    char* w = reinterpret_cast<char*>(ws);
    double* Sp = reinterpret_cast<double*>(w + l.Sp);
    int* tab = reinterpret_cast<int*>(w + l.tab);
    hipError_t e = hipMemsetAsync(Sp, 0, (size_t)K * f.nslab * 4 * sizeof(double), s);
    if (e != hipSuccess) return -(int)e;
    hipLaunchKernelGGL(tabx_kernel, dim3(1), dim3(256), 0, s, cov, D, f.nslab, tab);
    BEER_LAUNCH_CHECK();
    const int64_t tiles = (nframes + kAxFT - 1) / kAxFT;
    const float* Xt;
    if (f.xt_reused) {
        Xt = reinterpret_cast<const float*>(reinterpret_cast<const char*>(Rimg) +
                                            packed_tiles_bytes(nframes, K));
    } else {
        float* image = reinterpret_cast<float*>(w + l.Xt);
        hipLaunchKernelGGL(xt_image_kernel, dim3((unsigned)tiles), dim3(256), 0, s, nframes, D, f.NX,
                           X, image);
        BEER_LAUNCH_CHECK();
        Xt = image;
    }
    float* Gt = nullptr;
    if (f.sr) {
        Gt = reinterpret_cast<float*>(w + l.Gt);
        const int spad = acc_sets_spad(S, G);
        hipLaunchKernelGGL(gt_image_kernel, dim3((unsigned)tiles, (unsigned)((spad + 63) / 64)),
                           dim3(256), 0, s, nframes, S, spad, SR, Gt);
        BEER_LAUNCH_CHECK();
    }
    const int chain = beer::option(BEER_OPT_AX_MAXFRAMES);
    const int64_t max_z = (nframes + 511) / 512, min_z = (nframes + chain - 1) / chain;
    const int64_t rounds = ((int64_t)f.gx * f.gy * min_z + 255) / 256;
    int64_t gz = rounds * 256 / ((int64_t)f.gx * f.gy);
    if (gz < min_z) gz = min_z;
    if (gz > max_z) gz = max_z;
    if (gz < 1) gz = 1;
    const FrameSplit z = frame_split(nframes, gz, kAxFT);
    const int64_t nyz = ((int64_t)f.gy * z.gz + 7) / 8 * 8;
    const AccxArgs a = {nframes, z.fpb, D, K, f.nslab, f.NX, f.gx, f.gy, (int)z.gz, f.lgG,
                        f.sx ? 1 : 0, f.band ? 1 : 0, Xt, reinterpret_cast<const unsigned*>(Rimg),
                        tab, Sp, Gt, dim3((unsigned)(nyz * f.gx)), f.lds, s};
    for (const auto& r : kAccxRows)
        if (r.sr == f.sr && r.NQ == f.NQ) {
            const int rc = r.launch(a);
            return rc != BEER_OK ? rc : unpackx(cov, D, K, Sp, acc, s);
        }
    return BEER_EINVAL;
}


bool supported_accf(int cov, int D, int S, int G) {
    return cov != BEER_FULL && D >= 1 && D <= 64 && S >= 1 && G >= 1 && G <= 256 &&
           nslab_of(cov, D) * 4 <= 160;
}

bool supported_frame_image(int cov, int D) {
    if (cov == BEER_FULL || D < 1) return false;
    const int nk_used = (nslab_of(cov, D) + 7) / 8;
    return nk_used <= kImgMaxNK && 2 * d4_of(D) <= 4 * img_nqt(nk_used);
}
size_t frame_image_bytes(int cov, int64_t nframes, int D) {
    if (!supported_frame_image(cov, D) || nframes < 0) return 0;
    const int nk = nk16_of(cov, D), nk_used = (nslab_of(cov, D) + 7) / 8;
    const int64_t tiles = (nframes + 31) / 32;
    return (size_t)tiles * frame_image_tile_u4(nk_used, img_nqt(nk_used)) * 16 +
           up256((size_t)(nk + 1) * 8 * sizeof(int));
}
int frame_image(int cov, int64_t nframes, int D, const float* X, void* image, hipStream_t s) {
    if (!supported_frame_image(cov, D)) return BEER_EINVAL;
    if (nframes == 0) return BEER_OK;
    const int nk = nk16_of(cov, D), nslab = nslab_of(cov, D), nk_used = (nslab + 7) / 8;
    const int64_t tiles = (nframes + 31) / 32;
    int* tab = reinterpret_cast<int*>(reinterpret_cast<char*>(image) +
                                      (size_t)tiles * frame_image_tile_u4(nk_used, img_nqt(nk_used)) * 16);
    hipLaunchKernelGGL(tabx_kernel, dim3(1), dim3(256), 0, s, cov, D, (nk + 1) * 8, tab);
    const size_t lds = (size_t)(nk + 1) * 8 * sizeof(int) +
                       (size_t)4 * (32 * ld16_of(D) + (D + 2) * kAfXS) * sizeof(float);
    hipLaunchKernelGGL(frame_image_kernel, dim3((unsigned)((tiles + 3) / 4)), dim3(256), lds, s,
                       nframes, D, nk, nslab, img_nqt(nk_used), X, tab, reinterpret_cast<u4*>(image));
    BEER_LAUNCH_CHECK();
    return BEER_OK;
}

AccfForm accf_form(int cov, int D, int S, int G, bool have_image) {
    AccfForm f = {};
    f.rc = BEER_EINVAL;
    if (!supported_accf(cov, D, S, G)) return f;
    f.Gp = accf_group_pad(S, G);
    f.NTC = accf_ntc(cov, D);
    f.NQT = accf_nqt(cov, D);
    f.XP = f.NQT == 6 ? 5 : 8;
    f.nchunks = (S * f.Gp + 16 * f.NTC - 1) / (16 * f.NTC);
    auto reach = [&](int ns) {
        for (int c = 0; c < f.nchunks; ++c) {
            const int lo = c * 16 * f.NTC / f.Gp, hi = (c * 16 * f.NTC + 60) / f.Gp;
            if ((hi < S ? hi : S - 1) - (lo < S ? lo : S - 1) > ns - 1) return false;
        }
        return true;
    };
    f.blk = S >= 4 && reach(4);
    f.ns_img = f.blk ? 4 : (reach(16) ? 16 : 0);
    f.NKU = (nslab_of(cov, D) + 7) / 8;
    f.use_image = have_image && f.ns_img && f.NTC == 4 && supported_frame_image(cov, D);
    f.waves = f.use_image ? beer::option(BEER_OPT_ACCFI_WAVES)
                          : ((f.NTC == 4 && f.NQT == 6) ? 8 : 4);
    f.rc = BEER_OK;
    return f;
}

AccfLayout accf_layout(int cov, int D, int S, int G) {
    AccfLayout l = {};
    if (!supported_accf(cov, D, S, G)) return l;
    const int NTC = accf_ntc(cov, D), nk = nk16_of(cov, D);
    const int nchunks = (S * accf_group_pad(S, G) + 16 * NTC - 1) / (16 * NTC);
    const PtabLayout p = ptab_layout(nchunks, nk, NTC);
    l.tab = p.tab;
    l.c0 = p.c0;
    l.Sp = l.c0 + 1024;
    l.bytes = l.Sp + up256((size_t)S * G * nslab_of(cov, D) * 4 * sizeof(double));
    return l;
}
size_t accf_workspace_bytes(int cov, int D, int S, int G) { return accf_layout(cov, D, S, G).bytes; }

namespace {

struct AccfArgs {
    int64_t nframes, fpb;
    int D, K, S, G, Greal, nk, nslab;
    const float* X;
    const u4 *image, *P;
    const int* tab;
    const float *log_norm, *sr;
    double* Sp;
    const float* c0;
    dim3 grid;
    size_t lds;
    hipStream_t s;
};

template <int NKU, int W, int NS>
int launch_accfi(const AccfArgs& a) {
    (void)hipFuncSetAttribute(reinterpret_cast<const void*>(accfi_kernel<NKU, W, NS>),
                              hipFuncAttributeMaxDynamicSharedMemorySize, beer::kMaxDynLds);
    hipLaunchKernelGGL((accfi_kernel<NKU, W, NS>), a.grid, dim3(64 * W), a.lds, a.s, a.nframes, a.K,
                       a.S, a.G, a.Greal, a.nk, a.nslab, a.image, a.P, a.log_norm, a.sr, a.fpb, a.Sp,
                       a.c0);
    BEER_LAUNCH_CHECK();
    return BEER_OK;
}
template <int NQT, int W, bool BLK>
int launch_accf(const AccfArgs& a) {
    constexpr int XP = NQT == 6 ? 5 : 8;
    (void)hipFuncSetAttribute(reinterpret_cast<const void*>(accf_kernel<4, NQT, true, W, XP, BLK>),
                              hipFuncAttributeMaxDynamicSharedMemorySize, beer::kMaxDynLds);
    hipLaunchKernelGGL((accf_kernel<4, NQT, true, W, XP, BLK>), a.grid, dim3(64 * W), a.lds, a.s,
                       a.nframes, a.D, a.K, a.S, a.G, a.Greal, a.nk, a.nslab, a.X, a.P, a.tab,
                       a.log_norm, a.sr, a.fpb, a.Sp, a.c0);
    BEER_LAUNCH_CHECK();
    return BEER_OK;
}
constexpr struct AccfiRow { int NKU, W, NS; int (*launch)(const AccfArgs&); } kAccfiRows[] = {
    {1, 8, 4, launch_accfi<1, 8, 4>},   {2, 8, 4, launch_accfi<2, 8, 4>},
    {3, 8, 4, launch_accfi<3, 8, 4>},   {4, 8, 4, launch_accfi<4, 8, 4>},
    {1, 8, 16, launch_accfi<1, 8, 16>}, {2, 8, 16, launch_accfi<2, 8, 16>},
    {3, 8, 16, launch_accfi<3, 8, 16>}, {4, 8, 16, launch_accfi<4, 8, 16>},
    {1, 4, 4, launch_accfi<1, 4, 4>},   {2, 4, 4, launch_accfi<2, 4, 4>},
    {3, 4, 4, launch_accfi<3, 4, 4>},   {4, 4, 4, launch_accfi<4, 4, 4>},
    {1, 4, 16, launch_accfi<1, 4, 16>}, {2, 4, 16, launch_accfi<2, 4, 16>},
    {3, 4, 16, launch_accfi<3, 4, 16>}, {4, 4, 16, launch_accfi<4, 4, 16>}};
constexpr struct { int NQT; bool blk; int (*launch)(const AccfArgs&); } kAccfRows[] = {
    {6, true, launch_accf<6, 8, true>},   {6, false, launch_accf<6, 8, false>},
    {9, true, launch_accf<9, 4, true>},   {9, false, launch_accf<9, 4, false>},
    {10, true, launch_accf<10, 4, true>}, {10, false, launch_accf<10, 4, false>}};

}

int acc_fused_bf16x3(int cov, int64_t nframes, int D, int S, int G, const float* X,
                     const float* expT, const float* logw, const float* log_norm,
                     const float* sr, const void* image, double* acc, void* ws, size_t ws_bytes,
                     hipStream_t s) {
    const AccfForm f = accf_form(cov, D, S, G, image != nullptr);
    const AccfLayout l = accf_layout(cov, D, S, G);
    if (f.rc != BEER_OK || ws_bytes < l.bytes) return BEER_EINVAL;
    const int Kreal = S * G, K = S * f.Gp, NTC = f.NTC, nk = nk16_of(cov, D);
    const int nchunks = f.nchunks, kpad = nchunks * NTC * 16;
    const int nslab = nslab_of(cov, D), nq = nslab * 4;
    char* w = reinterpret_cast<char*>(ws);
    void* P = w + l.P;
    int* tab = reinterpret_cast<int*>(w + l.tab);
    float* c0 = reinterpret_cast<float*>(w + l.c0);
    double* Sp = reinterpret_cast<double*>(w + l.Sp);
    hipError_t e = hipMemsetAsync(Sp, 0, (size_t)Kreal * nq * sizeof(double), s);
    if (e != hipSuccess) return -(int)e;
    hipLaunchKernelGGL(const_max_kernel, dim3(1), dim3(256), 0, s, cov, D, Kreal, expT, logw, c0);
    hipLaunchKernelGGL(packx_kernel, dim3(kpad), dim3(256),
                       (size_t)stats_dim(cov, D) * sizeof(float), s, cov, D, Kreal, NTC, expT, logw,
                       reinterpret_cast<unsigned short*>(P), tab, G, f.Gp, c0, 0);
    BEER_LAUNCH_CHECK();
    const int waves = f.waves;
    const int rounds = beer::option(BEER_OPT_ACCF_ROUNDS);
    int64_t gz = ((waves == 8 ? 256 : 512) * rounds + nchunks - 1) / nchunks;
    gz = (gz + 7) / 8 * 8;
    const int64_t chain = nframes >= ((int64_t)4 << 20) ? kAfMaxFramesPerWave : kAfMaxFramesPerWave / 2;
    const int64_t min_z = (nframes + (int64_t)waves * chain - 1) / ((int64_t)waves * chain);
    const int64_t max_z = (nframes + 32 * waves - 1) / (32 * waves);
    if (gz > max_z) gz = max_z;
    if (gz < min_z) gz = min_z;
    if (gz < 1) gz = 1;
    const FrameSplit z = frame_split(nframes, gz, 32 * waves);
    const size_t lds_p = (size_t)f.NKU * NTC * kBlockU4 * 16;
    AccfArgs a = {nframes, z.fpb, D, K, S, f.Gp, G, nk, nslab, X,
                  reinterpret_cast<const u4*>(image), reinterpret_cast<const u4*>(P), tab, log_norm,
                  sr, Sp, c0, dim3(xcd_grid(z.gz, nchunks, nchunks)), 0, s};
    int rc = BEER_EINVAL;
    const size_t lds_red = (size_t)waves * 16 * 64 * sizeof(float);
    if (f.use_image) {
        const size_t lds_i = lds_p + (size_t)waves * 64 * f.ns_img * sizeof(float);
        a.lds = lds_i > lds_red ? lds_i : lds_red;
        for (const AccfiRow& r : kAccfiRows)
            if (r.NKU == f.NKU && r.W == (waves == 8 ? 8 : 4) && r.NS == (f.ns_img == 4 ? 4 : 16))
                rc = r.launch(a);
    } else {
        a.lds = lds_p + (size_t)(nk + 1) * 8 * sizeof(int) + (size_t)2 * f.NQT * 64 * sizeof(int) +
                (size_t)waves * (32 * ld16_of(D) + (D + 2) * kAfXS + (f.blk ? 256 : 0)) *
                    sizeof(float);
        if (a.lds < lds_red) a.lds = lds_red;
        for (const auto& r : kAccfRows)
            if (r.NQT == f.NQT && r.blk == f.blk) rc = r.launch(a);
    }
    return rc != BEER_OK ? rc : unpackx(cov, D, Kreal, Sp, acc, s);
}

#endif

}
```

beer_amd/csrc/estep_mfma.h:

```cpp
#pragma once

#include <hip/hip_runtime.h>
#include <stddef.h>
#include <stdint.h>

namespace beer_mfma {

constexpr int kMaxDimF32 = 96, kMaxDimF64 = 64;
constexpr int kMaxDimX = 128;
inline int max_dim(size_t elem) { return elem == 8 ? kMaxDimF64 : kMaxDimF32; }
bool supported_llh(int D, int S, int G, size_t elem = 4);
bool supported_acc(int D, int K, size_t elem = 4);
bool supported_llh_x(int D, int S, int G);
bool supported_acc_x(int D, int K);
size_t estep_workspace_bytes(size_t elem, int cov, int D, int S, int G);
size_t acc_workspace_bytes(int cov, int D, int K, size_t elem = 4);

struct FrameSplit {
    int64_t gz, fpb;
};
inline FrameSplit frame_split(int64_t nframes, int64_t gz, int tile) {
    int64_t fpb = (nframes + gz - 1) / gz;
    fpb = (fpb + tile - 1) / tile * tile;
    return {(nframes + fpb - 1) / fpb, fpb};
}

size_t estepx_workspace_bytes(int cov, int D, int S, int G);
bool supported_llh_split(int D, int S, int G);
int estep_bf16x3(int cov, int64_t T, int D, int S, int G, const float* X, const float* expT,
                 const float* logw, float* resps, float* log_norm, double* llh_sum, void* ws,
                 size_t ws_bytes, hipStream_t s, bool packed = false,
                 const void* frame_image = nullptr);

struct LlhForm {
    int NT, GQ, jw, gl, nchunks;
};
LlhForm llh_form(int S, int G);
struct LlhxForm {
    int rc;
    int NT, GQ, jw, gl, nchunks;
    int Gp;
    bool packed, lno, img, bl, narrow, lnfi8, lane_major;
    bool xt;
    bool lnfi;
    int nku, lnfi_g;
};
LlhxForm llhx_form(int cov, int D, int S, int G, bool resps, bool packed, bool image,
                   size_t ws_bytes);

struct AccForm {
    int rc;
    int NQ;
    bool has_sr;
    int gx, gy;
};
AccForm acc_form(size_t elem, int cov, int D, int K, bool has_sr);
struct AccLayout {
    size_t Sp, tab, bytes;
};
AccLayout acc_layout(size_t elem, int cov, int D, int K);

struct AccxForm {
    int rc;
    int NQ;
    bool sr;
    int lgG;
    bool sx;
    bool band;
    bool xt_reused;
    int nslab, NX, gx, gy;
    size_t lds;
};
AccxForm accx_form(int cov, int D, int K, int S, int G, bool sets);
struct AccxLayout {
    size_t Sp, tab, Xt, Gt, bytes;
};
AccxLayout accx_layout(int cov, int64_t T, int D, int K, int S, int G, bool sets);

struct AccfForm {
    int rc;
    int Gp;
    int NTC, NQT, XP, nchunks;
    bool blk;
    int ns_img;
    bool use_image;
    int waves, NKU;
};
AccfForm accf_form(int cov, int D, int S, int G, bool have_image);
struct AccfLayout {
    size_t P, tab, c0, Sp, bytes;
};
AccfLayout accf_layout(int cov, int D, int S, int G);

struct AccdForm {
    int rc;
    int NJ2, NC;
    bool partial;
};
AccdForm accd_form(int cov, int64_t T, int D, int K, size_t ws_bytes);
struct AccdLayout {
    size_t part, cpart, bytes;
};
AccdLayout accd_layout(int cov, int64_t T, int D, int K);

int unpack_resps(int64_t T, int K, const void* packed, float* resps, hipStream_t s);
int pack_resps(int64_t T, int D, int S, int G, const float* X, const float* R, const float* SR,
               void* packed, hipStream_t s);
size_t packed_resps_bytes(int64_t T, int D, int K);
size_t accx_workspace_bytes(int cov, int64_t T, int D, int K);
int acc_bf16x3_packed(int cov, int64_t T, int D, int K, const float* X, const void* Rimg,
                      double* acc, void* ws, size_t ws_bytes, hipStream_t s, int S = 1, int G = 0,
                      const float* SR = nullptr);
bool supported_llh_packed_sets(int cov, int D, int S, int G);
bool supported_acc_sets(int cov, int D, int S, int G);
size_t accxs_workspace_bytes(int cov, int64_t T, int D, int S, int G);

bool supported_accf(int cov, int D, int S, int G);
size_t accf_workspace_bytes(int cov, int D, int S, int G);
int acc_fused_bf16x3(int cov, int64_t T, int D, int S, int G, const float* X, const float* expT,
                     const float* logw, const float* log_norm, const float* sr, const void* image,
                     double* acc, void* ws, size_t ws_bytes, hipStream_t s);
size_t frame_image_bytes(int cov, int64_t T, int D);
int frame_image(int cov, int64_t T, int D, const float* X, void* image, hipStream_t s);

bool supported_acc_diag(int cov, int64_t T, int D, int K);
size_t acc_diag_workspace_bytes(int cov, int64_t T, int D, int K);
int acc_diag_bf16x3(int cov, int64_t T, int D, int K, const float* X, const float* W, double* acc,
                    void* ws, size_t ws_bytes, hipStream_t s);

int estep_f32(int cov, int64_t T, int D, int S, int G, const float* X, const float* expT,
              const float* logw, float* resps, float* log_norm, double* llh_sum, void* ws,
              size_t ws_bytes, hipStream_t s);
int estep_f64(int cov, int64_t T, int D, int S, int G, const double* X, const double* expT,
              const double* logw, double* resps, double* log_norm, double* llh_sum, void* ws,
              size_t ws_bytes, hipStream_t s);
int acc_f32(int cov, int64_t T, int D, int S, int G, const float* X, const float* R,
            const float* SR, double* acc, void* ws, size_t ws_bytes, hipStream_t s);
int acc_f64(int cov, int64_t T, int D, int S, int G, const double* X, const double* R,
            const double* SR, double* acc, void* ws, size_t ws_bytes, hipStream_t s);

}
```

beer_amd/inference/batch.py:

```python

import os
import threading

import torch

from .. import _hip, hmm_kernels as hk, kernels
from ..models.gaussians import NormalSet
from ..models.mixtures import Mixture, MixtureSet, TiedMixtureSet
from ..models.modelset import JointModelSet
from ..models.sequence import HMM, BigramPhoneLoop, PhoneLoop
from ..models.vae import VAE
from ..stats import FrameStats
from .objectives import EvidenceLowerBoundInstance

__all__ = ['accumulate_elbo', 'pack_utterances', 'decode_batch', 'sample_paths_batch',
           'ShardStatics']

_SCRATCH_CAP = 48 << 30
_scratch_bytes = [int(os.environ['BEER_SCRATCH_GB']) << 30 if 'BEER_SCRATCH_GB' in os.environ
                  else None]


def _scratch_budget():
    if _scratch_bytes[0] is None:
        try:
            free, _ = torch.cuda.mem_get_info()
            _scratch_bytes[0] = max(1 << 28, min(_SCRATCH_CAP, free // 8))
        except Exception:
            _scratch_bytes[0] = _SCRATCH_CAP
    return _scratch_bytes[0]


class ShardStatics:

    def __init__(self):
        self.key, self.items, self.lengths, self.mark = None, {}, None, None

    def bind(self, lengths):
        n = len(lengths)
        mark = (n, lengths[0], lengths[n // 2], lengths[-1]) if n else (0,)
        if self.lengths is not lengths or self.mark != mark:
            if self.mark != mark or self.lengths != lengths:
                self.key, self.items = None, {}
            self.lengths, self.mark = lengths, mark

    def entry(self, key, name, make):
        if self.key != key:
            self.key, self.items = key, {}
        if name not in self.items:
            self.items[name] = make()
        return self.items[name]


def _capturing():
    return torch.cuda.is_available() and torch.cuda.is_current_stream_capturing()


def pack_utterances(utterances):
    if isinstance(utterances, tuple) and len(utterances) == 2 and \
            isinstance(utterances[0], torch.Tensor):
        X, lengths = utterances
        if not (isinstance(lengths, list) and set(map(type, lengths)) <= {int}):
            lengths = [int(n) for n in lengths]
        return _hip.on_device(X), lengths
    utterances = list(utterances)
    lengths = [len(u) for u in utterances]
    dev = _hip.require_device()
    X = torch.cat([u.to(dev) for u in utterances], dim=0).contiguous()
    return X, lengths


def _groups(emissions):
    if isinstance(emissions, JointModelSet):
        out = []
        for m in emissions.modelsets:
            out += _groups(m)
        return out
    if isinstance(emissions, MixtureSet):
        return [(emissions, len(emissions), emissions.n_leaves_per_mixture)]
    if isinstance(emissions, TiedMixtureSet):
        return [(emissions, len(emissions), len(emissions.modelset))]
    if isinstance(emissions, NormalSet):
        return [(emissions, len(emissions), 1)]
    raise NotImplementedError(f'unsupported emission model {type(emissions).__name__}')


def _normalset(group):
    return group.normalset if isinstance(group, (MixtureSet, TiedMixtureSet)) else group


def _n_gaussians(group, S, G):
    return G if isinstance(group, TiedMixtureSet) else S * G


def _sub_batches(lengths, bytes_per_frame, max_frames):
    budget = max(1, min(max_frames, _scratch_budget() // max(1, bytes_per_frame)))
    total = sum(lengths)
    n_runs = max(1, -(-total // budget))
    target = -(-total // n_runs)
    runs, cur, n = [], [], 0
    for u, T in enumerate(lengths):
        if cur and (n + T > budget or (n >= target and len(runs) < n_runs - 1)):
            runs.append(cur)
            cur, n = [], 0
        cur.append(u)
        n += T
    if cur:
        runs.append(cur)
    return runs


_local = threading.local()


def _throttle(depth=2):
    if _capturing():
        return torch.cuda.Event()
    in_flight = _local.__dict__.setdefault('in_flight', [])
    while len(in_flight) >= depth:
        in_flight.pop(0).synchronize()
    ev = torch.cuda.Event()
    in_flight.append(ev)
    return ev


def _cached_batch(graph, run_lengths, dtype):
    cache = graph.__dict__.setdefault('_batch_cache', {})
    key = (dtype, tuple(run_lengths))
    dg = graph.device_graph(dtype)
    hit = cache.get(key)
    if hit is not None and hit.dgraphs[0] is dg:
        return hit
    if len(cache) >= 8:
        cache.clear()
    batch = hk.HmmBatch([graph], [0] * len(run_lengths), run_lengths, dtype)
    cache[key] = batch
    return batch


_KL_BESIDE = os.environ.get('BEER_KL_SIDE_STREAM', '1') != '0'


def _kl_beside_the_estep(model, device):
    if not _KL_BESIDE or isinstance(model, VAE) or device.type != 'cuda' or _capturing():
        return torch.as_tensor(model.kl_div_posterior_prior()), None
    main = torch.cuda.current_stream(device)
    for param in model.bayesian_parameters():
        for dist in (getattr(param, 'posterior', None), getattr(param, 'prior', None)):
            if dist is not None and hasattr(dist, 'expected_sufficient_statistics'):
                dist.expected_sufficient_statistics()
                dist.log_norm()
                dist.natural_parameters()
    side_streams = _local.__dict__.setdefault('side_streams', {})
    side = side_streams.get(device)
    if side is None:
        side = side_streams[device] = torch.cuda.Stream(device)
    side.wait_stream(main)
    with torch.cuda.stream(side):
        kl = torch.as_tensor(model.kl_div_posterior_prior())
        done = side.record_event()
    return kl, done


def _finish(model, value_terms, kl, nutt, acc, datasize, total_frames):
    value = value_terms - float(nutt) * kl.to(value_terms.device, torch.float64)
    return EvidenceLowerBoundInstance(value, acc, model.bayesian_parameters(),
                                      total_frames, datasize)


def _like(param, t):
    return t.to(dtype=param.stats.dtype, device=param.stats.device)


def _mixture_batch(model, X, lengths, datasize, labels, max_frames, statics=None):
    ns = model.normalset
    K, cov = len(ns), ns.cov_type
    dev, dtype = X.device, X.dtype
    exp_T = ns.means_precisions.natural_form()
    lw = model._log_weights().view(1, K)
    Q = FrameStats(X[:1], cov).shape[1]
    acc = torch.zeros(K, Q, dtype=torch.float64, device=dev)
    utt_llh = torch.zeros(len(lengths), dtype=torch.float64, device=dev)

    def offsets_and_scales():
        off = torch.zeros(len(lengths) + 1, dtype=torch.int64)
        off[1:] = torch.cumsum(torch.as_tensor(lengths, dtype=torch.int64), 0)
        up = _hip.upload({'off': off, 'scales': torch.as_tensor(
            [datasize / float(T) for T in lengths], dtype=torch.float64)}, dev)
        return off, up['off'], up['scales']
    statics = statics if statics is not None else ShardStatics()
    statics.bind(lengths)
    skey = ('mixture', len(lengths), float(datasize), str(dev))
    off, off_dev, scales = statics.entry(skey, 'offsets', offsets_and_scales)
    lab_dev = None if labels is None else \
        _hip.on_device(torch.as_tensor(labels)).to(torch.int64).contiguous()
    if lab_dev is not None and model.nested:
        M = len(model.modelset)
        lw_sets = model.modelset.leaf_log_weights()
    for run in _sub_batches(lengths, K * X.element_size(), max_frames):
        done = _throttle()
        f0, f1 = int(off[run[0]]), int(off[run[-1] + 1])
        stats = FrameStats(X[f0:f1], cov)
        lab = None if lab_dev is None else lab_dev[f0:f1]
        wide = kernels.wide_mixture_split(stats, K, cov) if lab is None else None
        seg = off_dev[run[0]:run[-1] + 2] - f0
        if lab is not None and model.nested:
            set_norm, resps = kernels.mixtureset_estep(stats, exp_T, lw_sets, M, K // M, cov)
            onehot = torch.zeros_like(set_norm).scatter_(1, lab.view(-1, 1), 1.)
            hk.segment_sum(kernels.rowdot(set_norm, onehot), seg, len(run),
                           out=utt_llh[run[0]:run[-1] + 1])
            kernels.normal_accumulate(stats, resps, onehot, M, K // M, cov, acc=acc)
            done.record()
            continue
        if lab is None and kernels.packed_path_ok(stats, K, cov):
            log_norm, resps = kernels.mixture_estep_packed(stats, exp_T, lw, K, cov)
        elif wide:
            log_norm, resps = kernels.wide_mixture_estep(stats, exp_T, lw, K, cov, wide)
        else:
            log_norm, resps = kernels.mixtureset_estep(stats, exp_T, lw, 1, K, cov, labels=lab)
        hk.segment_sum(log_norm.view(-1), seg, len(run), out=utt_llh[run[0]:run[-1] + 1])
        kernels.normal_accumulate(stats, resps, None, K, 1, cov, acc=acc)
        done.record()
    value_terms = (scales * utt_llh).sum()
    out = {**model._weights_accumulate(acc), ns.means_precisions: _like(ns.means_precisions, acc)}
    return value_terms, out


def _emission_estep(groups, stats, dtype, for_accumulate=False):
    cols, comps = [], []
    for grp, S, G in groups:
        ns = _normalset(grp)
        gstats = stats.as_cov(ns.cov_type)
        if isinstance(grp, TiedMixtureSet):
            tied = grp.estep(gstats)
            cols.append(tied[2])
            comps.append(('tied',) + tied)
            continue
        lw = grp.leaf_log_weights() if isinstance(grp, MixtureSet) else None
        fused = for_accumulate and G > 1 and \
            kernels.fused_accumulate_ok(gstats, S, G, ns.cov_type)
        if for_accumulate and G > 1 and not fused and \
                kernels.packed_sets_ok(gstats, S, G, ns.cov_type):
            log_norm, packed = kernels.mixtureset_estep_packed(
                gstats, ns.means_precisions.natural_form(), lw, S, G, ns.cov_type)
            cols.append(log_norm)
            comps.append(packed)
            continue
        log_norm, resps = kernels.mixtureset_estep(
            gstats, ns.means_precisions.natural_form(), lw, S, G, ns.cov_type,
            want_resps=for_accumulate and G > 1 and not fused)
        cols.append(log_norm)
        comps.append(('fused', log_norm, lw) if fused else resps)
    pc_all = cols[0] if len(cols) == 1 else torch.cat(cols, dim=-1)
    return pc_all, comps


def _hmm_batch(model, X, lengths, datasize, graphs, scale, viterbi, state_paths, max_frames,
               frame_images=None, statics=None, sample=None):
    emissions = model._emissions()
    groups = _groups(emissions)
    S_total = sum(S for _, S, _ in groups)
    dev, dtype = X.device, X.dtype
    free_loop = graphs is None
    accs, tied_counts = [], []
    for grp, S, G in groups:
        ns = _normalset(grp)
        Q = FrameStats(X[:1], ns.cov_type).shape[1]
        accs.append(torch.zeros(_n_gaussians(grp, S, G), Q, dtype=torch.float64, device=dev))
        tied_counts.append(torch.zeros(S, G, dtype=torch.float64, device=dev)
                      if isinstance(grp, TiedMixtureSet) else None)
    nutt = len(lengths)
    utt_llh = torch.zeros(nutt, dtype=torch.float64, device=dev)

    def offsets_and_scales():
        off = torch.zeros(nutt + 1, dtype=torch.int64)
        off[1:] = torch.cumsum(torch.as_tensor(lengths, dtype=torch.int64), 0)
        return off, _hip.to_device(torch.as_tensor([datasize / float(T) for T in lengths],
                                                   dtype=torch.float64), dev)
    statics = statics if statics is not None else ShardStatics()
    statics.bind(lengths)
    skey = ('hmm', nutt, float(datasize), str(dev))
    off, scales = statics.entry(skey, 'offsets', offsets_and_scales)
    xi_tot = g0_tot = flow_tot = None
    learned = model.transitions is not None
    if learned and not free_loop:
        model._bound_set(graphs).refresh(dtype)
    tcounts_tot = None
    bigram = free_loop and isinstance(model, BigramPhoneLoop)
    counts_tot = None
    max_S = model.graph.n_states if free_loop else max(g.n_states for g in graphs)
    K_scratch = sum(2 * G if isinstance(grp, TiedMixtureSet) else S * G
                    for grp, S, G in groups
                    if isinstance(grp, TiedMixtureSet) or (G > 1 and not kernels.fused_accumulate_ok(
                        FrameStats(X, _normalset(grp).cov_type), S, G, _normalset(grp).cov_type)))
    bpf = (K_scratch + 2 * S_total) * X.element_size() + max_S * (3 * X.element_size() + 8)
    if sample is not None:
        bpf += 16
    if bigram:
        model.declare_block()
        bpf += 16 * len(model.start_pdf)
    if frame_images is None or not frame_images.covers(X):
        bpf += max((_hip.lib().beer_frame_image_bytes(
            _hip.COV_CODE[_normalset(grp).cov_type], 1 << 20, X.shape[1]) >> 20)
            for grp, _, _ in groups) if X.dtype == torch.float32 else 0
    runs = statics.entry(skey, ('runs', bpf, max_frames), lambda: [
        (run, int(off[run[0]]), int(off[run[-1] + 1]), [lengths[u] for u in run])
        for run in _sub_batches(lengths, bpf, max_frames)])
    for run_index, (run, f0, f1, run_lengths) in enumerate(runs):
        done = _throttle()
        stats = FrameStats(X[f0:f1], _normalset(groups[0][0]).cov_type, images=frame_images)
        pc_all, comps = _emission_estep(groups, stats, dtype, for_accumulate=True)
        if free_loop:
            batch = _cached_batch(model.graph, run_lengths, dtype)
        else:
            def images_of(uniq):
                sets, out = {}, []
                for g in uniq:
                    owner = getattr(g, '_set', None)
                    if owner is None:
                        out.append(g.device_graph(dtype))
                    elif id(owner) not in sets:
                        sets[id(owner)] = True
                        out.append(owner.device_image(dtype)[0])
                return out

            def make_batch():
                uniq, ids, seen = [], [], {}
                for u in run:
                    g = graphs[u]
                    if id(g) not in seen:
                        seen[id(g)] = len(uniq)
                        uniq.append(g)
                    ids.append(seen[id(g)])
                return hk.HmmBatch(uniq, ids, run_lengths, dtype), graphs, uniq, images_of(uniq)
            bkey = ('batch', run_index, bpf, max_frames, id(graphs), len(graphs),
                    id(graphs[run[0]]), id(graphs[run[-1]]), str(dtype))
            batch, _, uniq, images = statics.entry(skey, bkey, make_batch)
            if not all(a is b for a, b in zip(images, images_of(uniq))):
                statics.items.pop(bkey)
                batch, _, uniq, images = statics.entry(skey, bkey, make_batch)
        hard = viterbi or state_paths is not None or sample is not None
        if bigram and not hard:
            sr, counts = hk.posteriors_bigram(batch, pc_all, scale,
                                              utt_llh=utt_llh[run[0]:run[-1] + 1])
            counts_tot = counts if counts_tot is None else counts_tot + counts
            _accumulate_emissions(groups, comps, accs, sr, stats, tied_counts)
            done.record()
            continue
        need_counts = free_loop and isinstance(model, PhoneLoop)
        hubbed = need_counts and getattr(getattr(batch.dgraphs[0], 'lowdeg', None), 'n_hubs', 0) >= 1
        if learned and not hard and hk.fused_ok(batch) and (hubbed or not need_counts):
            sr, g0, flow, tc = hk.posteriors_fused(batch, pc_all, scale, want_counts=need_counts,
                                                   utt_llh=utt_llh[run[0]:run[-1] + 1],
                                                   want_transitions=True)
            xi = None
        elif learned and not hard:
            pc_llhs = hk.gather(batch, pc_all, scale)
            gamma, g0, flow, xi, tc = hk.forward_backward_counts(batch, pc_llhs)
            sr, _ = hk.scatter(batch, pc_llhs, gamma, S_total, scale, want_exp_llh=False,
                               utt_llh=utt_llh[run[0]:run[-1] + 1])
        elif not hard and hk.fused_ok(batch) and (hubbed or not need_counts):
            sr, g0, flow = hk.posteriors_fused(batch, pc_all, scale, want_counts=need_counts,
                                               utt_llh=utt_llh[run[0]:run[-1] + 1])
            xi = None
        else:
            pc_llhs = hk.gather(batch, pc_all, scale)
            if hard:
                if sample is not None:
                    path = hk.sample_paths(batch, pc_llhs, None if sample is True
                                           else sample.reshape(1, -1)[:, f0:f1])[0]
                elif state_paths is None:
                    path = hk.viterbi(batch, pc_llhs)
                else:
                    path = torch.cat([torch.as_tensor(state_paths[u]).reshape(-1) for u in run])
                gamma, xi, g0 = hk.path_posteriors(batch, path, want_xi=free_loop)
                flow = None
                if learned:
                    tc = hk.path_counts(batch, path, xi)
            else:
                gamma, xi, g0, _, flow = hk.forward_backward(batch, pc_llhs, want_xi=free_loop)
            sr, _ = hk.scatter(batch, pc_llhs, gamma, S_total, scale, want_exp_llh=False,
                               utt_llh=utt_llh[run[0]:run[-1] + 1])
        if learned:
            tc = model.transition_counts(batch.dgraphs[0], tc)
            tcounts_tot = tc if tcounts_tot is None else tcounts_tot + tc
        if free_loop:
            if xi is not None:
                xi_tot = xi if xi_tot is None else xi_tot + xi
            if g0 is not None:
                g0_tot = g0 if g0_tot is None else g0_tot + g0
            if flow is not None:
                flow_tot = flow if flow_tot is None else flow_tot + flow
        _accumulate_emissions(groups, comps, accs, sr, stats, tied_counts)
        done.record()
    value_terms = (scales * utt_llh).sum()
    out = {}
    for (grp, S, G), acc, cnt in zip(groups, accs, tied_counts):
        ns = _normalset(grp)
        out[ns.means_precisions] = _like(ns.means_precisions, acc)
        if isinstance(grp, MixtureSet):
            out.update(grp.weights_accumulate(acc))
        elif isinstance(grp, TiedMixtureSet):
            out.update(grp.weights_accumulate(cnt))
    if learned:
        out.update(model.transitions.accumulate_counts(tcounts_tot))
    if isinstance(model, BigramPhoneLoop):
        if bigram and counts_tot is None and xi_tot is not None:
            counts_tot = model.bigram_counts(xi_tot)
        out.update(model.weights_accumulate(counts_tot if bigram else None))
    if isinstance(model, PhoneLoop):
        wparam = model.categorical.mean_field_factorization()[0][0]
        ref = wparam.stats
        if free_loop:
            counts = model.phone_counts(xi_tot, g0_tot, flow_tot).to(dtype=ref.dtype,
                                                                     device=ref.device)
            cstats = model.categorical.sufficient_statistics(counts.view(1, -1))
            out.update(model.categorical.accumulate(cstats))
        else:
            fake = torch.zeros(len(model.start_pdf), dtype=ref.dtype, device=ref.device)
            out.update(model.categorical.accumulate(fake[None, :]))
    return value_terms, out


def _accumulate_emissions(groups, comps, accs, sr, stats, counts=None):
    first = 0
    for n, ((grp, S, G), comp, acc) in enumerate(zip(groups, comps, accs)):
        ns = _normalset(grp)
        sr_g = sr if len(groups) == 1 else sr[:, first:first + S].contiguous()
        first += S
        gstats = stats.as_cov(ns.cov_type)
        if isinstance(grp, TiedMixtureSet):
            r, _ = kernels.tied_accumulate(*comp[1:], sr_g, counts=counts[n])
            kernels.normal_accumulate(gstats, r, None, G, 1, ns.cov_type, acc=acc)
        elif G == 1:
            kernels.normal_accumulate(gstats, sr_g, None, S, 1, ns.cov_type, acc=acc)
        elif isinstance(comp, tuple):
            kernels.mixtureset_accumulate_fused(
                gstats, ns.means_precisions.natural_form(), comp[2], comp[1], sr_g, S, G,
                ns.cov_type, acc=acc)
        else:
            kernels.normal_accumulate(gstats, comp, sr_g, S, G, ns.cov_type, acc=acc)


def _vae_batch(model, X, lengths, datasize, nsamples, llh_weight, kl_weight):
    kwargs = {'utt_lengths': lengths} if isinstance(model.prior, HMM) else {}
    broadcast, model.reference_broadcast = model.reference_broadcast, False
    try:
        per_frame = model.expected_log_likelihood(X, nsamples=nsamples, llh_weight=llh_weight,
                                                  kl_weight=kl_weight, **kwargs)
    finally:
        model.reference_broadcast = broadcast
    w = [float(datasize) if broadcast else datasize / float(T) for T in lengths]
    weights = torch.repeat_interleave(
        torch.as_tensor(w, dtype=torch.float64, device=per_frame.device),
        torch.as_tensor(lengths, device=per_frame.device))
    value_terms = (weights * per_frame.to(torch.float64)).sum()
    return value_terms, model.accumulate(None)


def accumulate_elbo(model, utterances, datasize=-1, inference_graphs=None, scale=1.,
                    viterbi=False, state_paths=None, labels=None, max_frames=1 << 24,
                    nsamples=1, llh_weight=1., kl_weight=1., frame_images=None, statics=None,
                    sample=False):
    if sample is not None and sample is not False:
        packed = isinstance(utterances, tuple) and len(utterances) == 2 and \
            isinstance(utterances[0], torch.Tensor)
        if not packed:
            utterances = list(utterances)
        sample = hk.check_sample(sample, sum(int(n) for n in utterances[1]) if packed
                                 else sum(len(u) for u in utterances), viterbi, state_paths)
        if not isinstance(model, HMM):
            raise ValueError('sample: HMM models only')
    else:
        sample = None
    X, lengths = pack_utterances(utterances)
    if any(T <= 0 for T in lengths):
        raise ValueError('empty utterance in the batch')
    total = sum(lengths)
    if datasize <= 0:
        datasize = total
    if len(lengths) == 0:
        return EvidenceLowerBoundInstance(0., {}, [], 0, datasize)
    kl, kl_done = _kl_beside_the_estep(model, X.device)
    if isinstance(model, Mixture):
        value_terms, acc = _mixture_batch(model, X, lengths, datasize, labels, max_frames, statics)
    elif isinstance(model, HMM):
        value_terms, acc = _hmm_batch(model, X, lengths, datasize, inference_graphs, scale,
                                      viterbi, state_paths, max_frames, frame_images, statics,
                                      sample)
    elif isinstance(model, VAE):
        value_terms, acc = _vae_batch(model, X, lengths, datasize, nsamples, llh_weight,
                                      kl_weight)
    else:
        raise NotImplementedError(f'no batched E-step for {type(model).__name__}')
    model.clear_cache()
    if kl_done is not None:
        torch.cuda.current_stream(X.device).wait_event(kl_done)
    return _finish(model, value_terms, kl, len(lengths), acc, datasize, total)


def decode_batch(model, utterances, inference_graphs=None, scale=1., max_frames=1 << 20):
    return _paths_batch(model, utterances, inference_graphs, scale, max_frames, 0,
                        lambda batch, pc_llhs: hk.viterbi(batch, pc_llhs, map_pdf=True))


def sample_paths_batch(model, utterances, inference_graphs=None, scale=1., nsamples=1,
                       generator=None, max_frames=1 << 20):
    nsamples = int(nsamples)
    if nsamples < 1:
        raise ValueError('sample_paths_batch: at least one sample')
    return _paths_batch(model, utterances, inference_graphs, scale, max_frames, 16 * nsamples,
                        lambda batch, pc_llhs: hk.sample_paths(
                            batch, pc_llhs, nsamples=nsamples, generator=generator, map_pdf=True),
                        trellis_bytes=8)


def _paths_batch(model, utterances, inference_graphs, scale, max_frames, extra_bytes, search,
                 trellis_bytes=4):
    X, lengths = pack_utterances(utterances)
    groups = _groups(model._emissions())
    S_total = sum(S for _, S, _ in groups)
    K_max = sum(2 * G if isinstance(grp, TiedMixtureSet) else S * G for grp, S, G in groups)
    off = [0]
    for T in lengths:
        off.append(off[-1] + T)
    paths = []
    max_S = model.graph.n_states if inference_graphs is None \
        else max(g.n_states for g in inference_graphs)
    if inference_graphs is not None and len(inference_graphs) and \
            getattr(getattr(inference_graphs[0], '_set', None), 'is_bound', False):
        model._bound_set(inference_graphs).refresh(X.dtype)
    bpf = (K_max + S_total) * X.element_size() + max_S * (X.element_size() + trellis_bytes) + \
        extra_bytes
    for run in _sub_batches(lengths, bpf, max_frames):
        f0, f1 = off[run[0]], off[run[-1] + 1]
        stats = FrameStats(X[f0:f1], _normalset(groups[0][0]).cov_type)
        pc_all, _ = _emission_estep(groups, stats, X.dtype)
        run_lengths = [lengths[u] for u in run]
        if inference_graphs is None:
            batch = hk.HmmBatch([model.graph], [0] * len(run), run_lengths, X.dtype)
        else:
            uniq, ids, seen = [], [], {}
            for u in run:
                g = inference_graphs[u]
                if id(g) not in seen:
                    seen[id(g)] = len(uniq)
                    uniq.append(g)
                ids.append(seen[id(g)])
            batch = hk.HmmBatch(uniq, ids, run_lengths, X.dtype)
        path = search(batch, hk.gather(batch, pc_all, scale))
        paths += list(torch.split(path, run_lengths, dim=-1))
    return paths
```

beer_amd/inference/objectives.py:

```python

import threading

import torch

from .. import _hip
from ..hmm_kernels import check_sample, segment_sum

__all__ = ['evidence_lower_bound', 'EvidenceLowerBoundInstance']


def add_acc_stats(acc_stats1, acc_stats2):
    out = dict(acc_stats1)
    for key, val in acc_stats2.items():
        out[key] = out[key] + val if key in out else val
    return out


def scale_acc_stats(acc_stats, scale):
    return {key: scale * val for key, val in acc_stats.items()}


class EvidenceLowerBoundInstance:

    def __init__(self, value, acc_stats, model_parameters, minibatchsize, datasize):
        self.value = value
        self._acc_stats = acc_stats
        self._model_parameters = set(model_parameters)
        self._minibatchsize = minibatchsize
        self._datasize = datasize

    def __repr__(self):
        return f'EvidenceLowerBoundInstance(value={self.value})'

    def __float__(self):
        value = self.value
        return float(value.detach() if isinstance(value, torch.Tensor) else value)

    def __add__(self, other):
        if not isinstance(other, EvidenceLowerBoundInstance):
            raise ValueError('EvidenceLowerBoundInstance')
        if self._datasize != other._datasize:
            raise ValueError('Cannot add ELBOs evaluated on different data set')
        return EvidenceLowerBoundInstance(
            self.value + other.value,
            add_acc_stats(self._acc_stats, other._acc_stats),
            self._model_parameters.union(other._model_parameters),
            self._minibatchsize + other._minibatchsize,
            self._datasize)

    def backward(self, std_params=True):
        if std_params and isinstance(self.value, torch.Tensor) and self.value.requires_grad:
            (-self.value).backward()
        scale = self._datasize / self._minibatchsize
        for parameter in self._model_parameters:
            try:
                parameter.store_stats(scale * self._acc_stats[parameter])
            except KeyError:
                pass

    def sync(self, model):
        self._model_parameters = set(model.bayesian_parameters())


_span_lock = threading.Lock()
_spans = {}


def _span(n, device):
    key = (device, n)
    with _span_lock:
        off = _spans.get(key)
        if off is None:
            if len(_spans) >= 64:
                _spans.clear()
            off = _spans[key] = torch.tensor([0, n], dtype=torch.int64, device=device)
    return off


def frame_sum(values):
    values = _hip.on_device(values).reshape(-1)
    return segment_sum(values, _span(values.numel(), values.device), 1)[0]


def evidence_lower_bound(model=None, minibatch_data=None, datasize=-1, **kwargs):
    if model is None and minibatch_data is None and datasize > 0:
        return EvidenceLowerBoundInstance(0., {}, [], 0, datasize)
    if model is None or minibatch_data is None:
        raise ValueError('if datasize is not provided, need at least "model" '
                         'and "minibatch_data"')
    mb_datasize = len(minibatch_data)
    if datasize <= 0:
        datasize = mb_datasize
    scale = datasize / float(mb_datasize)
    if 'sample' in kwargs:
        check_sample(kwargs['sample'], mb_datasize, kwargs.get('viterbi', False),
                     kwargs.get('state_path'))
    stats = model.sufficient_statistics(minibatch_data)
    exp_llh = model.expected_log_likelihood(stats, **kwargs)
    kl_div = torch.as_tensor(model.kl_div_posterior_prior())
    if isinstance(exp_llh, torch.Tensor) and exp_llh.requires_grad:
        total = _hip.on_device(exp_llh).to(torch.float64).sum()
    else:
        total = frame_sum(exp_llh)
    elbo_value = float(scale) * total - kl_div.to(total.device, torch.float64)
    acc_stats = model.accumulate(stats)
    model.clear_cache()
    return EvidenceLowerBoundInstance(elbo_value, acc_stats, model.bayesian_parameters(),
                                      mb_datasize, datasize)
```

beer_amd/kernels.py:

```python

import functools
import os

import torch

from . import _hip
from .stats import FrameStats

__all__ = ['normal_llh', 'mixtureset_estep', 'normal_accumulate', 'weights_from_acc',
           'tied_lognorm', 'tied_accumulate',
           'is_dense', 'dense_llh', 'dense_softmax', 'dense_accumulate', 'rowdot',
           'attach_stats_grad', 'differentiable_stats', 'sample_stats', 'attach_frame_grad',
           'frames_llh_backward', 'normal_llh_autograd']

LOG_2PI = 1.8378770664093453


def is_dense(stats):
    return isinstance(stats, torch.Tensor)


def _exact(X):
    return X.dtype == torch.float32 and not _hip.f32_fast_ok(X)


def _frames(stats):
    if not isinstance(stats, FrameStats):
        raise TypeError('expected the lazy statistics returned by '
                        'model.sufficient_statistics(X)')
    return stats


def normal_llh(stats, exp_stats, cov_type):
    st = _frames(stats)
    X = st.data
    T, D = X.shape
    E = _hip.on_device(exp_stats, X.dtype)
    K = E.shape[0]
    if st.scale == 1.0:
        return mixtureset_estep(st, E, None, K, 1, cov_type, want_resps=False)[0]
    out = torch.empty(T, K, dtype=X.dtype, device=X.device)
    _hip.call('beer_mixtureset_estep', _hip.dtype_code(X.dtype), _hip.COV_CODE[cov_type],
              T, D, K, 1, _hip.ptr(X), _hip.ptr(E), None, None, st.scale,
              _hip.ptr(out), None, None, None, None, 0)
    return out


@functools.lru_cache(maxsize=4096)
def estep_buffers(dtype_code, cov, D, S, G, args, ws_bytes):
    def refused(entry, mask):
        return _hip.estep_route(entry, dtype_code, cov, D, S, G, mask, ws_bytes) == _hip.EINVAL
    need_resps = bool(args & _hip.ARG_RESPS)
    if not need_resps and refused(_hip.ESTEP_PLAIN, args):
        need_resps = True
    if need_resps and refused(_hip.ESTEP_PLAIN, args | _hip.ARG_RESPS):
        raise _hip.HipInvalid('beer_mixtureset_estep failed: invalid argument')
    return need_resps, not refused(_hip.ESTEP_IMAGE, args)


def mixtureset_estep(stats, exp_stats, log_weights, S, G, cov_type, labels=None,
                     want_resps=True, llh_sum=None):
    st = _frames(stats)
    X = st.data
    T, D = X.shape
    E = _hip.on_device(exp_stats, X.dtype)
    lw = None if log_weights is None else _hip.on_device(log_weights, X.dtype)
    K = S * G
    if E.shape[0] != K:
        raise ValueError(f'{E.shape[0]} Gaussians for {S} x {G} mixture components')
    code, cov = _hip.dtype_code(X.dtype, _exact(X)), _hip.COV_CODE[cov_type]
    ws, ws_bytes = _hip.workspace('beer_estep_workspace_bytes', X.dtype, cov, D, S, G, X.device)
    args = _hip.ARG_LOG_NORM | (_hip.ARG_RESPS if want_resps else 0) | \
        (0 if llh_sum is None else _hip.ARG_LLH_SUM) | (0 if lw is None else _hip.ARG_LOG_WEIGHTS) | \
        (0 if labels is None else _hip.ARG_LABELS) | (_hip.ARG_SCALED if st.scale != 1.0 else 0)
    need_resps, image_ok = estep_buffers(code, cov, D, S, G, args, ws_bytes)
    log_norm = torch.empty(T, S, dtype=X.dtype, device=X.device)
    img = st.frame_image(cov_type) if image_ok else None
    if img is not None:
        _hip.call('beer_mixtureset_lognorm_image', cov, T, D, S, G, _hip.ptr(X), _hip.ptr(E),
                  _hip.ptr(lw), _hip.ptr(img), _hip.ptr(log_norm), _hip.ptr(llh_sum),
                  _hip.ptr(ws), ws_bytes)
        return log_norm, None
    resps = torch.empty(T, K, dtype=X.dtype, device=X.device) if need_resps else None
    lab = None
    if labels is not None:
        lab = _hip.on_device(torch.as_tensor(labels)).to(torch.int64).contiguous()
    _hip.call('beer_mixtureset_estep', code, cov, T, D, S, G, _hip.ptr(X), _hip.ptr(E),
              _hip.ptr(lw), _hip.ptr(lab), st.scale, None, _hip.ptr(log_norm), _hip.ptr(resps),
              _hip.ptr(llh_sum), _hip.ptr(ws), ws_bytes)
    return log_norm, resps if want_resps else None


class PackedResps:

    def __init__(self, words, nframes, ncomp):
        self.words, self.shape = words, (nframes, ncomp)

    def unpack(self):
        T, K = self.shape
        out = torch.empty(T, K, dtype=torch.float32, device=self.words.device)
        _hip.call('beer_unpack_resps', T, K, _hip.ptr(self.words), _hip.ptr(out))
        return out


def packed_path_ok(stats, K, cov_type):
    st = _frames(stats)
    X = st.data
    if st.scale != 1.0 or not _hip.f32_fast_ok(X):
        return False
    code, D = _hip.COV_CODE[cov_type], X.shape[1]
    lib, dt = _hip.lib(), _hip.dtype_code(X.dtype)
    return lib.beer_estep_workspace_bytes(dt, code, D, 1, K) > 0 and \
        lib.beer_accumulate_packed_workspace_bytes(code, X.shape[0], D, K) > 0


def mixture_estep_packed(stats, exp_stats, log_weights, K, cov_type, llh_sum=None):
    st = _frames(stats)
    X = st.data
    T, D = X.shape
    E = _hip.on_device(exp_stats, X.dtype)
    lw = _hip.on_device(log_weights, X.dtype)
    if E.shape[0] != K or lw.numel() != K:
        raise ValueError(f'{E.shape[0]} Gaussians, {lw.numel()} weights for {K} components')
    log_norm = torch.empty(T, 1, dtype=X.dtype, device=X.device)
    words = torch.empty(_hip.lib().beer_packed_resps_bytes(T, D, K) // 4, dtype=torch.int32,
                        device=X.device)
    ws, ws_bytes = _hip.workspace('beer_estep_workspace_bytes', X.dtype,
                                  _hip.COV_CODE[cov_type], D, 1, K, X.device)
    _hip.call('beer_mixture_estep_packed', _hip.COV_CODE[cov_type], T, D, K, _hip.ptr(X),
              _hip.ptr(E), _hip.ptr(lw), _hip.ptr(log_norm), _hip.ptr(words), _hip.ptr(llh_sum),
              _hip.ptr(ws), ws_bytes)
    return log_norm, PackedResps(words, T, K)


def packed_sets_ok(stats, S, G, cov_type):
    st = _frames(stats)
    X = st.data
    if st.scale != 1.0 or X.dtype != torch.float32 or not _hip.f32_fast_ok(X):
        return False
    return bool(_hip.lib().beer_mixtureset_packed_supported(_hip.COV_CODE[cov_type], X.shape[1],
                                                            S, G))


def mixtureset_estep_packed(stats, exp_stats, log_weights, S, G, cov_type, llh_sum=None):
    st = _frames(stats)
    X = st.data
    T, D = X.shape
    K = S * G
    E = _hip.on_device(exp_stats, X.dtype)
    lw = None if log_weights is None else _hip.on_device(log_weights, X.dtype)
    if E.shape[0] != K or (lw is not None and lw.numel() != K):
        raise ValueError(f'{E.shape[0]} Gaussians for {S} x {G} components')
    log_norm = torch.empty(T, S, dtype=X.dtype, device=X.device)
    words = torch.empty(_hip.lib().beer_packed_resps_bytes(T, D, K) // 4, dtype=torch.int32,
                        device=X.device)
    ws, ws_bytes = _hip.workspace('beer_estep_workspace_bytes', X.dtype,
                                  _hip.COV_CODE[cov_type], D, S, G, X.device)
    _hip.call('beer_mixtureset_estep_packed', _hip.COV_CODE[cov_type], T, D, S, G, _hip.ptr(X),
              _hip.ptr(E), _hip.ptr(lw), _hip.ptr(log_norm), _hip.ptr(words), _hip.ptr(llh_sum),
              _hip.ptr(ws), ws_bytes)
    return log_norm, PackedResps(words, T, K)



class WideResps:

    def __init__(self, stats, exp_stats, log_weights, split, cov_type, block_lse, block_resps,
                 packed, K=None):
        self.stats, self.exp_stats, self.log_weights = stats, exp_stats, log_weights
        self.split, self.cov_type = split, cov_type
        self.block_lse, self.block_resps, self.packed = block_lse, block_resps, packed
        self.K = split[0] * split[1] if K is None else K

    def dense(self):
        S2, G2 = self.split
        within = self.packed.unpack() if self.packed is not None else mixtureset_estep(
            self.stats, self.exp_stats, self.log_weights, S2, G2, self.cov_type)[1]
        return (within * self.block_resps.repeat_interleave(G2, dim=1))[:, :self.K]


def wide_mixture_split(stats, K, cov_type):
    st = _frames(stats)
    X = st.data
    if K <= 256 or st.scale != 1.0 or X.dtype != torch.float32 or not _hip.f32_fast_ok(X):
        return None
    ok = (lambda S2, G2: packed_sets_ok(st, S2, G2, cov_type)) if cov_type == 'full' else \
        (lambda S2, G2: fused_accumulate_ok(st, S2, G2, cov_type))
    first = -(-K // 256)
    for S2 in range(first, min(K // 8, first + 64) + 1):
        if K % S2 == 0 and ok(S2, K // S2):
            return S2, K // S2
    for G2 in ((128, 64) if cov_type == 'full' else (256, 128)):
        S2 = -(-K // G2)
        if ok(S2, G2):
            return S2, G2
    return None


def wide_mixture_estep(stats, exp_stats, log_weights, K, cov_type, split):
    S2, G2 = split
    st = _frames(stats)
    E = _hip.on_device(exp_stats, st.data.dtype)
    lw = _hip.on_device(log_weights, st.data.dtype).reshape(-1)
    pad = S2 * G2 - K
    if pad:
        E = torch.cat([E, E[:1].expand(pad, -1)]).contiguous()
        lw = torch.cat([lw, torch.full((pad,), -1.0e30, dtype=lw.dtype, device=lw.device)])
    lw = lw.reshape(S2, G2)
    packed = None
    if cov_type == 'full':
        lse, packed = mixtureset_estep_packed(st, E, lw, S2, G2, cov_type)
    else:
        lse, _ = mixtureset_estep(st, E, lw, S2, G2, cov_type, want_resps=False)
    log_norm, share = dense_softmax(lse, None, 1, S2)
    return log_norm, WideResps(st, E, lw, split, cov_type, lse, share, packed, K=K)


def pack_resps(stats, comp_resps, state_resps, S, G):
    st = _frames(stats)
    X = st.data
    T, D = X.shape
    K = S * G
    cr = _hip.on_device(comp_resps, X.dtype)
    sr = None if state_resps is None else _hip.on_device(state_resps, X.dtype)
    words = torch.empty(_hip.lib().beer_packed_resps_bytes(T, D, K) // 4, dtype=torch.int32,
                        device=X.device)
    _hip.call('beer_pack_resps', T, D, S, G, _hip.ptr(X), _hip.ptr(cr), _hip.ptr(sr),
              _hip.ptr(words))
    return PackedResps(words, T, K)


def _repack_pays(stats, K, cov_type):
    X = stats.data
    if cov_type != 'full' or stats.shape[1] <= 512 or K % 4 or stats.scale != 1.0 or \
            not _hip.f32_fast_ok(X):
        return False
    return _hip.lib().beer_accumulate_packed_workspace_bytes(
        _hip.COV_CODE[cov_type], X.shape[0], X.shape[1], K) > 0


def normal_accumulate(stats, comp_resps, state_resps, S, G, cov_type, acc=None):
    st = _frames(stats)
    if st.scale != 1.0:
        raise ValueError('scaled statistics cannot be accumulated')
    X = st.data
    T, D = X.shape
    K = S * G
    Q = st.shape[1]
    if acc is None:
        acc = torch.zeros(K, Q, dtype=torch.float64, device=X.device)
    if isinstance(comp_resps, WideResps):
        wr = comp_resps
        S2, G2 = wr.split
        if state_resps is not None or wr.K != K or wr.stats.data.data_ptr() != X.data_ptr():
            raise ValueError('factored responsibilities: one mixture, the frames they came from')
        full = acc if S2 * G2 == K else torch.zeros(S2 * G2, Q, dtype=torch.float64, device=X.device)
        if wr.packed is not None:
            normal_accumulate(st, wr.packed, wr.block_resps, S2, G2, cov_type, acc=full)
        else:
            mixtureset_accumulate_fused(st, wr.exp_stats, wr.log_weights, wr.block_lse,
                                        wr.block_resps, S2, G2, cov_type, acc=full)
        if full is not acc:
            acc += full[:K]
        return acc
    if isinstance(comp_resps, PackedResps) and state_resps is not None:
        if tuple(comp_resps.shape) != (T, K) or not packed_sets_ok(st, S, G, cov_type):
            raise ValueError('packed responsibilities of a mixture set: same frames and '
                             'components, a shape with `packed_sets_ok`')
        sr = _hip.on_device(state_resps, X.dtype)
        if tuple(sr.shape) != (T, S):
            raise ValueError(f'state responsibilities {tuple(sr.shape)}, expected {(T, S)}')
        code = _hip.COV_CODE[cov_type]
        ws, ws_bytes = _hip.packed_workspace(code, T, D, K, X.device, sets=(S, G))
        _hip.call('beer_mixtureset_accumulate_packed', code, T, D, S, G, _hip.ptr(X),
                  _hip.ptr(comp_resps.words), _hip.ptr(sr), _hip.ptr(acc), _hip.ptr(ws), ws_bytes)
        return acc
    if isinstance(comp_resps, PackedResps):
        if tuple(comp_resps.shape) != (T, K):
            raise ValueError('packed responsibilities: same frames and components')
        ws, ws_bytes = _hip.packed_workspace(_hip.COV_CODE[cov_type], T, D, K, X.device)
        _hip.call('beer_normal_accumulate_packed', _hip.COV_CODE[cov_type], T, D, K,
                  _hip.ptr(X), _hip.ptr(comp_resps.words), _hip.ptr(acc), _hip.ptr(ws), ws_bytes)
        return acc
    if comp_resps is not None and X.dtype == torch.float32 and _repack_pays(st, K, cov_type):
        return normal_accumulate(st, pack_resps(st, comp_resps, state_resps, S, G), None, S, G,
# ... 336 lines not shown
```

include/beer_hip.h:

```cpp
#ifndef BEER_HIP_H
#define BEER_HIP_H

#include <stddef.h>
#include <stdint.h>

#ifdef __cplusplus
extern "C" {
#endif

#define BEER_F32 0
#define BEER_F64 1
#define BEER_I16 2

#define BEER_FULL 0
#define BEER_DIAG 1
#define BEER_ISO 2

#define BEER_OK 0
#define BEER_EINVAL (-100000)

int beer_hip_version(void);
int beer_hip_device_count(void);

#define BEER_OPT_AX_MAXFRAMES 0
#define BEER_OPT_ACCF_ROUNDS 1
#define BEER_OPT_ACCFI_WAVES 2
#define BEER_OPT_LNFI 3
#define BEER_OPT_FB_LOG 4
#define BEER_OPT_K1_LDS 5
#define BEER_OPT_COUNT 6
int beer_hip_set_option(int option, int value);
int beer_hip_get_option(int option);

#define BEER_EXACT 0x10


int beer_nw_expected_stats(int dtype, int K, int D, const void* mean,
                           const void* scale, const void* scale_matrix,
                           const void* dof, void* out, void* stream);
int beer_nw_expected_stats_log_norm(int dtype, int K, int D, const void* mean,
                                    const void* scale, const void* scale_matrix,
                                    const void* dof, void* out, void* log_norm,
                                    void* stream);
int beer_nw_log_norm(int dtype, int K, int D, const void* mean,
                     const void* scale, const void* scale_matrix,
                     const void* dof, void* out, void* stream);
int beer_nw_natural(int dtype, int K, int D, const void* mean,
                    const void* scale, const void* scale_matrix,
                    const void* dof, void* out, void* stream);
int beer_nw_from_natural(int dtype, int K, int D, const void* eta, void* mean,
                         void* scale, void* scale_matrix, void* dof,
                         void* stream);

int beer_nw_update(int dtype, int K, int D, const void* eta, void* mean, void* scale,
                   void* scale_matrix, void* dof, void* exp_stats, void* log_norm,
                   void* moments, void* stream);

int beer_ng_expected_stats(int dtype, int K, int D, const void* mean,
                           const void* scale, const void* shape,
                           const void* rates, void* out, void* stream);
int beer_ng_log_norm(int dtype, int K, int D, const void* mean,
                     const void* scale, const void* shape, const void* rates,
                     void* out, void* stream);
int beer_ng_natural(int dtype, int K, int D, const void* mean,
                    const void* scale, const void* shape, const void* rates,
                    void* out, void* stream);
int beer_ng_from_natural(int dtype, int K, int D, const void* eta, void* mean,
                         void* scale, void* shape, void* rates, void* stream);

int beer_ing_expected_stats(int dtype, int K, int D, const void* mean,
                            const void* scale, const void* shape,
                            const void* rate, void* out, void* stream);
int beer_ing_log_norm(int dtype, int K, int D, const void* mean,
                      const void* scale, const void* shape, const void* rate,
                      void* out, void* stream);
int beer_ing_natural(int dtype, int K, int D, const void* mean,
                     const void* scale, const void* shape, const void* rate,
                     void* out, void* stream);
int beer_ing_from_natural(int dtype, int K, int D, const void* eta, void* mean,
                          void* scale, void* shape, void* rate, void* stream);

int beer_dirichlet_expected_stats(int dtype, int S, int G, const void* conc,
                                  void* out, void* stream);
int beer_dirichlet_log_norm(int dtype, int S, int G, const void* conc,
                            void* out, void* stream);
int beer_dirichlet_natural(int dtype, int S, int G, const void* conc,
                           void* out, void* stream);
int beer_dirichlet_from_natural(int dtype, int S, int G, const void* eta,
                                void* conc, void* stream);
int beer_sb_transform_stats(int dtype, int P, const void* counts, int64_t* ordering,
                            void* stats, void* stream);
int beer_sb_log_weights(int dtype, int P, const void* conc, const int64_t* ordering,
                        void* log_w, void* log_1_v_sum, void* stream);
int beer_sb_set_log_weights(int dtype, int n, int K, const void* conc, const int64_t* ordering,
                            void* log_w, void* stream);
int beer_sb_set_transform_stats(int dtype, int n, int K, const void* counts,
                                const int64_t* ordering, void* stats, void* stream);
int beer_dirichlet_log_weights(int dtype, int S, int G, const void* conc,
                               void* out, void* stream);

int beer_gamma_expected_stats(int dtype, int n, const void* shape,
                              const void* rate, void* out, void* stream);
int beer_gamma_log_norm(int dtype, int n, const void* shape, const void* rate,
                        void* out , void* stream);
int beer_gamma_natural(int dtype, int n, const void* shape, const void* rate,
                       void* out, void* stream);
int beer_gamma_from_natural(int dtype, int n, const void* eta, void* shape,
                            void* rate, void* stream);

int beer_kl_div(int dtype, int K, int Q, const void* exp_stats_q,
                const void* eta_q, const void* eta_p, const void* lnorm_q,
                const void* lnorm_p, void* out, void* stream);

int beer_natural_grad_step(int dtype, int64_t n, const void* eta_prior,
                           const void* eta_post, const void* stats,
                           double lrate, void* out, void* stream);

int beer_suffstats_expand(int dtype, int cov, int64_t T, int D, const void* X,
                          void* out, void* stream);


int beer_mixtureset_estep(int dtype, int cov, int64_t T, int D, int S, int G,
                          const void* X, const void* exp_stats,
                          const void* log_weights, const int64_t* labels,
                          double stat_scale, void* pc_llh, void* log_norm,
                          void* comp_resps, double* llh_sum, void* workspace,
                          size_t workspace_bytes, void* stream);

size_t beer_estep_workspace_bytes(int dtype, int cov, int D, int S, int G);
size_t beer_accumulate_workspace_bytes(int dtype, int cov, int D, int S, int G);
size_t beer_accumulate_frames_workspace_bytes(int dtype, int cov, int64_t T, int D, int S, int G);

int beer_normal_accumulate(int dtype, int cov, int64_t T, int D, int S, int G,
                           const void* X, const void* comp_resps,
                           const void* state_resps, double* acc, void* workspace,
                           size_t workspace_bytes, void* stream);

size_t beer_packed_resps_bytes(int64_t T, int D, int K);
size_t beer_accumulate_packed_workspace_bytes(int cov, int64_t T, int D, int K);
int beer_mixture_estep_packed(int cov, int64_t T, int D, int K, const float* X,
                              const float* exp_stats, const float* log_weights,
                              float* log_norm, void* packed_resps, double* llh_sum,
                              void* workspace, size_t workspace_bytes, void* stream);
int beer_normal_accumulate_packed(int cov, int64_t T, int D, int K, const float* X,
                                  const void* packed_resps, double* acc,
                                  void* workspace, size_t workspace_bytes,
                                  void* stream);
int beer_mixtureset_packed_supported(int cov, int D, int S, int G);
size_t beer_mixtureset_accumulate_packed_workspace_bytes(int cov, int64_t T, int D, int S,
                                                         int G);
int beer_mixtureset_estep_packed(int cov, int64_t T, int D, int S, int G, const float* X,
                                 const float* exp_stats, const float* log_weights,
                                 float* log_norm, void* packed_resps, double* llh_sum,
                                 void* workspace, size_t workspace_bytes, void* stream);
int beer_mixtureset_accumulate_packed(int cov, int64_t T, int D, int S, int G,
                                      const float* X, const void* packed_resps,
                                      const float* state_resps, double* acc,
                                      void* workspace, size_t workspace_bytes,
                                      void* stream);
int beer_pack_resps(int64_t T, int D, int S, int G, const float* X,
                    const float* comp_resps, const float* state_resps,
                    void* packed_resps, void* stream);
int beer_unpack_resps(int64_t T, int K, const void* packed_resps, float* resps,
                      void* stream);

size_t beer_accumulate_fused_workspace_bytes(int cov, int D, int S, int G);
int beer_mixtureset_accumulate_fused(int cov, int64_t T, int D, int S, int G,
                                     const float* X, const float* exp_stats,
                                     const float* log_weights, const float* log_norm,
                                     const float* state_resps, const void* frame_image,
                                     double* acc, void* workspace, size_t workspace_bytes,
                                     void* stream);

size_t beer_frame_image_bytes(int cov, int64_t T, int D);
int beer_mixtureset_lognorm_image(int cov, int64_t T, int D, int S, int G, const float* X,
                                  const float* exp_stats, const float* log_weights,
                                  const void* frame_image, float* log_norm, double* llh_sum,
                                  void* workspace, size_t workspace_bytes, void* stream);
int beer_frame_image(int cov, int64_t T, int D, const float* X, void* image,
                     size_t image_bytes, void* stream);

#define BEER_ESTEP_PLAIN 0
#define BEER_ESTEP_PACKED 1
#define BEER_ESTEP_IMAGE 2
#define BEER_ARG_PC_LLH 1u
#define BEER_ARG_LOG_NORM 2u
#define BEER_ARG_RESPS 4u
#define BEER_ARG_LLH_SUM 8u
#define BEER_ARG_LABELS 16u
#define BEER_ARG_SCALED 32u
#define BEER_ARG_LOG_WEIGHTS 64u
#define BEER_ESTEP_GENERIC 0x10000000
#define BEER_ESTEP_EXACT_F32 0x20000000
#define BEER_ESTEP_EXACT_F64 0x30000000
#define BEER_ESTEP_LLHX 0x40000000
#define BEER_ESTEP_LNFI 0x50000000
#define BEER_ESTEP_FAMILY(route) ((route) & 0x70000000)
#define BEER_ESTEP_GENERIC_PASS1 1
#define BEER_ESTEP_GENERIC_FUSED 2
#define BEER_ESTEP_GENERIC_NORMALISE 3
#define BEER_ESTEP_GENERIC_LABELS 4
#define BEER_ESTEP_X_PACKED 0x100
#define BEER_ESTEP_X_LNO 0x200
#define BEER_ESTEP_X_IMG 0x400
#define BEER_ESTEP_X_BL 0x800
#define BEER_ESTEP_X_NARROW 0x1000
#define BEER_ESTEP_X_LANE_MAJOR 0x2000
#define BEER_ESTEP_X_PADDED 0x4000
#define BEER_ESTEP_X_XT 0x8000
int beer_estep_route(int entry, int dtype, int cov, int D, int S, int G, unsigned args,
                     size_t workspace_bytes);

#define BEER_ACC_PLAIN 0
#define BEER_ACC_PACKED 1
#define BEER_ACC_FUSED 2
#define BEER_ARG_STATE_RESPS 128u
#define BEER_ARG_IMAGE 256u
#define BEER_ACC_GENERIC 0x10000000
#define BEER_ACC_EXACT_F32 0x20000000
#define BEER_ACC_EXACT_F64 0x30000000
#define BEER_ACC_DIAG 0x40000000
#define BEER_ACC_ACCX 0x50000000
#define BEER_ACC_ACCF 0x60000000
#define BEER_ACC_FAMILY(route) ((route) & 0x70000000)
#define BEER_ACC_SR 0x100
#define BEER_ACC_D_PARTIAL 0x200
#define BEER_ACC_X_SX 0x200
#define BEER_ACC_X_XT_REUSED 0x400
#define BEER_ACC_F_BLK 0x200
#define BEER_ACC_F_IMAGE 0x400
int beer_accumulate_route(int entry, int dtype, int cov, int64_t T, int D, int S, int G,
                          unsigned args, size_t workspace_bytes);

int beer_weights_from_acc(int S, int G, int Q, const double* acc,
                          double* out , void* stream);

int beer_tied_lognorm(int dtype, int64_t T, int K, int S, const void* l, const double* lw,
                      void* pc, void* m, int64_t* log_count, void* stream);
int beer_tied_accumulate(int dtype, int64_t T, int K, int S, const void* l, const void* m,
                         const void* pc, const double* lw, const void* g, void* r, double* C,
                         void* stream);


#define BEER_SEG 8
typedef struct {
    int32_t n_states;
    int32_t n_arcs;
    int32_t n_in_seg;
    int32_t n_out_seg;
    const void* init;
    const void* final;
    const int32_t* in_ptr;
    const int32_t* in_src;
    const int32_t* in_dst;
    const void* in_w;
    const int32_t* in_seg;
    const int32_t* in_row_seg;
    const int32_t* out_ptr;
    const int32_t* out_dst;
    const int32_t* out_src;
    const void* out_w;
    const int32_t* out_seg;
    const int32_t* out_row_seg;
    const struct beer_graph_lowdeg* lowdeg;
} beer_graph;

typedef struct beer_graph_lowdeg {
    int32_t n_arcs;
    int32_t n_hubs;
    const int32_t* in_ptr;
    const int32_t* in_src;
    const void* in_w;
    const int32_t* out_ptr;
    const int32_t* out_dst;
    const void* out_w;
    const int32_t* hub_src_id;
    const void* hub_src_w;
    const int32_t* hub_dst_id;
    const void* hub_dst_w;
    const int32_t* src_ptr;
    const int32_t* src_list;
    const int32_t* dst_ptr;
    const int32_t* dst_list;
} beer_graph_lowdeg;

typedef struct {
    int32_t nutt;
    int32_t max_states;
    int32_t max_arcs;
    int32_t max_segs;
    int32_t all_lowdeg;
    int32_t n_graphs;
    const int64_t* frame_off;
    const int64_t* llh_off;
    const int32_t* graph_id;
    const beer_graph* graphs;
    const int32_t* pdf_off;
    const int32_t* pdf_ids;
    int32_t max_degree;
    int32_t max_hubs;
// ... 263 lines not shown
```

Baseline: 269.5 million.

## Fuse mixture E-step/accumulate handover and add single-kernel stats tail

For a single mixture, the E-step pack kernel now computes its own constant maximum and zeroes the accumulator slabs and table, so the separate const-max kernel, memset and table kernel are skipped. The accumulate step then writes raw sums, and a new tail kernel turns them into scaled stats, weight stats, per-utterance log-likelihoods and the ELBO value in one launch, using a ticket-based last-block reduction. The aim is to remove several small launches and host-side torch ops per VB iteration. In exchange it adds a more complex workspace layout and atomic ticket synchronisation, and it only applies when the handover conditions hold.

```diff
diff --git a/beer_amd/_hip.py b/beer_amd/_hip.py
--- a/beer_amd/_hip.py
+++ b/beer_amd/_hip.py
@@ -158,6 +158,9 @@
 def estep_route(entry, dtype_code_, cov, D, S, G, args, workspace_bytes):
     return lib().beer_estep_route(entry, dtype_code_, cov, D, S, G, args, workspace_bytes)
 
+
+HANDOVER_PRIME = HANDOVER_PRIMED = 0x100
+HANDOVER_SUMS = 0x200
 
 ACC_PLAIN, ACC_PACKED, ACC_FUSED = 0, 1, 2
 ARG_STATE_RESPS, ARG_IMAGE = 128, 256
@@ -263,6 +266,8 @@
     'beer_mixture_estep_packed': [c_i, c_l, c_i, c_i, c_p, c_p, c_p, c_p, c_p, c_p, c_p, c_z,
                                   c_p],
     'beer_normal_accumulate_packed': [c_i, c_l, c_i, c_i, c_p, c_p, c_p, c_p, c_z, c_p],
+    'beer_mixture_tail': [c_i, c_i, c_i, ctypes.c_int32, c_p, c_p, c_p, c_p, c_p, c_d, c_p, c_p,
+                          c_p, c_p, c_p, c_p, c_p, c_z, c_p],
     'beer_mixtureset_estep_packed': [c_i, c_l, c_i, c_i, c_i, c_p, c_p, c_p, c_p, c_p, c_p, c_p,
                                      c_z, c_p],
     'beer_mixtureset_accumulate_packed': [c_i, c_l, c_i, c_i, c_i, c_p, c_p, c_p, c_p, c_p, c_z,
@@ -350,6 +355,8 @@
     'beer_accumulate_packed_workspace_bytes': [c_i, c_l, c_i, c_i],
     'beer_mixtureset_accumulate_packed_workspace_bytes': [c_i, c_l, c_i, c_i, c_i],
     'beer_hmm_fb_scratch_doubles': [c_i, c_p, c_i],
+    'beer_handover_workspace_offset': [c_i, c_i, c_i],
+    'beer_mixture_tail_scratch_bytes': [ctypes.c_int32],
     'beer_frames_llh_backward_workspace_bytes': [c_i, c_i, c_l, c_i, c_i],
 }
 
diff --git a/beer_amd/csrc/estep.hip b/beer_amd/csrc/estep.hip
--- a/beer_amd/csrc/estep.hip
+++ b/beer_amd/csrc/estep.hip
@@ -451,14 +451,15 @@
 
 int estepx_entry(int entry, bool set, int cov, int64_t T, int D, int S, int G, const float* X,
                  const float* exp_stats, const float* logw, const void* image, float* log_norm,
-                 void* resps, double* llh_sum, void* ws, size_t ws_bytes, void* stream) {
+                 void* resps, double* llh_sum, void* ws, size_t ws_bytes, void* stream,
+                 void* prime_acc_ws = nullptr) {
     const unsigned args = (log_norm ? BEER_ARG_LOG_NORM : 0u) | (resps ? BEER_ARG_RESPS : 0u) |
                           (llh_sum ? BEER_ARG_LLH_SUM : 0u) | (logw ? BEER_ARG_LOG_WEIGHTS : 0u);
     const int rc = estepx_refusal(entry, set, cov, D, S, G, args, ws ? ws_bytes : 0);
     if (rc != BEER_OK || T == 0) return rc;
     return beer_mfma::estep_bf16x3(cov, T, D, S, G, X, exp_stats, logw, (float*)resps, log_norm,
                                    llh_sum, ws, ws_bytes, as_stream(stream),
-                                   entry == BEER_ESTEP_PACKED, image);
+                                   entry == BEER_ESTEP_PACKED, image, prime_acc_ws);
 }
 
 int accx_refusal(bool set, int cov, int64_t T, int D, int S, int G, size_t ws_bytes) {
@@ -611,18 +612,58 @@
                               void* packed_resps, double* llh_sum, void* workspace,
                               size_t workspace_bytes, void* stream) {
     BEER_REQUIRE(T >= 0 && X && exp_stats);
+    const bool prime = (cov & BEER_HANDOVER_PRIME) != 0;
+    cov &= ~BEER_HANDOVER_PRIME;
+    if (!prime)
+        return estepx_entry(BEER_ESTEP_PACKED, false, cov, T, D, 1, K, X, exp_stats, log_weights,
+                            nullptr, log_norm, packed_resps, llh_sum, workspace, workspace_bytes,
+                            stream);
+    const size_t off = beer_handover_workspace_offset(cov, D, K);
+    BEER_REQUIRE(off > 0 && workspace && workspace_bytes >= off && T > 0);
+    BEER_REQUIRE(accx_refusal(false, cov, T, D, 1, K, workspace_bytes - off) == BEER_OK);
     return estepx_entry(BEER_ESTEP_PACKED, false, cov, T, D, 1, K, X, exp_stats, log_weights, nullptr,
-                        log_norm, packed_resps, llh_sum, workspace, workspace_bytes, stream);
+                        log_norm, packed_resps, llh_sum, workspace, off, stream,
+                        static_cast<char*>(workspace) + off);
 }
 
 int beer_normal_accumulate_packed(int cov, int64_t T, int D, int K, const float* X,
                                   const void* packed_resps, double* acc, void* workspace,
                                   size_t workspace_bytes, void* stream) {
-    BEER_REQUIRE(X && packed_resps && acc && workspace);
+    const bool primed = (cov & BEER_HANDOVER_PRIMED) != 0, sums = (cov & BEER_HANDOVER_SUMS) != 0;
+    cov &= ~(BEER_HANDOVER_PRIMED | BEER_HANDOVER_SUMS);
+    BEER_REQUIRE(X && packed_resps && workspace && (acc != nullptr) != sums);
     BEER_REQUIRE(accx_refusal(false, cov, T, D, 1, K, workspace_bytes) == BEER_OK);
+    BEER_REQUIRE(T > 0 || !(primed || sums));
     if (T == 0) return BEER_OK;
     return beer_mfma::acc_bf16x3_packed(cov, T, D, K, X, packed_resps, acc, workspace,
-                                        workspace_bytes, as_stream(stream));
+                                        workspace_bytes, as_stream(stream), 1, 0, nullptr, primed);
+}
+
+size_t beer_handover_workspace_offset(int cov, int D, int K) {
+    const size_t own = beer_estep_workspace_bytes(BEER_F32, cov, D, 1, K);
+    return (own + 255) / 256 * 256;
+}
+
+int beer_mixture_tail(int cov, int D, int K, int32_t n_utts, const void* sums,
+                      const float* log_norm, const int64_t* frame_off, const double* utt_scale,
+                      const float* kl, double stat_scale, float* stats, float* stats_scaled,
+                      float* weight_stats, float* weight_stats_scaled, double* utt_llh,
+                      double* value, void* scratch, size_t scratch_bytes, void* stream) {
+    BEER_REQUIRE(cov >= 0 && cov <= 2 && D >= 1 && K >= 1 && n_utts >= 1);
+    BEER_REQUIRE(sums && log_norm && frame_off && utt_scale && stats && stats_scaled &&
+                 weight_stats && weight_stats_scaled && utt_llh && value && scratch);
+    BEER_REQUIRE(beer_mfma::accx_form(cov, D, K, 1, K, false).rc == BEER_OK);
+    BEER_REQUIRE(scratch_bytes >= beer_mixture_tail_scratch_bytes(n_utts));
+    beer_mfma::MixtureTail t = {cov, D, K, n_utts, static_cast<const double*>(sums), log_norm,
+                                frame_off, utt_scale, kl, stat_scale, stats, stats_scaled,
+                                weight_stats, weight_stats_scaled, utt_llh,
+                                reinterpret_cast<double*>(static_cast<char*>(scratch) + 16),
+                                static_cast<unsigned*>(scratch), value};
+    return beer_mfma::mixture_tail(t, as_stream(stream));
+}
+
+size_t beer_mixture_tail_scratch_bytes(int32_t n_utts) {
+    return n_utts < 1 ? 0 : 16 + (size_t)n_utts * sizeof(double);
 }
 
 int beer_mixtureset_packed_supported(int cov, int D, int S, int G) {
diff --git a/beer_amd/csrc/estep_bf16.hip b/beer_amd/csrc/estep_bf16.hip
--- a/beer_amd/csrc/estep_bf16.hip
+++ b/beer_amd/csrc/estep_bf16.hip
@@ -115,15 +115,47 @@
     if (threadIdx.x == 0) c0[0] = m > -1.0e300 ? (float)m : 0.f;
 }
 
+struct AccPrime {
+    double* Sp;
+    size_t n;
+    int* tab;
+    int nslab;
+};
+
 __global__ __launch_bounds__(256) void packx_kernel(int cov, int D, int K, int NT,
                                                     const float* __restrict__ E,
                                                     const float* __restrict__ logw,
                                                     unsigned short* __restrict__ P,
                                                     int* __restrict__ tab, int G, int Gp,
-                                                    const float* __restrict__ c0, int lane_major) {
+                                                    float* __restrict__ c0, int lane_major,
+                                                    int own_c0, AccPrime prime) {
     extern __shared__ __attribute__((aligned(16))) char pack_lds[];
+    __shared__ double red[8];
     const int nk = nk16_of(cov, D), nent = nk * 32;
     const int slot = blockIdx.x;
+    double c0v;
+    if (own_c0) {
+        const int Q = stats_dim(cov, D);
+        double m = -1.0e300;
+        for (int kc = threadIdx.x; kc < K; kc += blockDim.x) {
+            const double v = const_total(cov, D, E + (size_t)kc * Q, logw ? (double)logw[kc] : 0.0);
+            if (v == v && v > m && v < 1.0e300) m = v;
+        }
+        m = block_max(m, red);
+        const float c = m > -1.0e300 ? (float)m : 0.f;
+        if (slot == 0 && threadIdx.x == 0) c0[0] = c;
+        c0v = (double)c;
+    } else {
+        c0v = (double)c0[0];
+    }
+    if (prime.Sp) {
+        for (size_t i = (size_t)slot * blockDim.x + threadIdx.x; i < prime.n;
+             i += (size_t)gridDim.x * blockDim.x)
+            prime.Sp[i] = 0.0;
+        if (slot == 0)
+            for (int s = threadIdx.x; s < prime.nslab; s += blockDim.x)
+                prime.tab[s] = slabx_entry(cov, D, s);
+    }
     const int k = slot % Gp < G ? (slot / Gp) * G + slot % Gp : K;
     const int chunk = slot / (NT * 16), kk = slot % (NT * 16);
     const int c = lane_major ? kk % NT : 4 * (kk / 64) + (kk % 4);
@@ -154,7 +186,7 @@
         } else if (q % 4 == 0) {
             const bool last = q / 4 == nslab - 1;
             const double want = k < K ? const_share(cov, D, q / 4, rowl, logw ? (double)logw[k] : 0.0) -
-                                            (last ? (double)c0[0] : 0.0)
+                                            (last ? c0v : 0.0)
                                       : (last ? kPadLogit : 0.0);
             const float hi = (float)want;
             const double rem = (want - (double)hi) * (1.0 / (double)kConstEps);
@@ -1966,9 +1998,19 @@
 
 int estep_bf16x3(int cov, int64_t nframes, int D, int S, int G, const float* X, const float* expT,
                  const float* logw, float* resps, float* log_norm, double* llh_sum, void* ws,
-                 size_t ws_bytes, hipStream_t s, bool packed, const void* image) {
+                 size_t ws_bytes, hipStream_t s, bool packed, const void* image,
+                 void* prime_acc_ws) {
     const LlhxForm f = llhx_form(cov, D, S, G, resps != nullptr, packed, image != nullptr, ws_bytes);
     if (f.rc != BEER_OK) return f.rc;
+    AccPrime prime = {};
+    if (prime_acc_ws) {
+        const AccxForm af = accx_form(cov, D, G, 1, G, false);
+        const AccxLayout al = accx_layout(cov, nframes, D, G, 1, G, false);
+        if (S != 1 || !packed || af.rc != BEER_OK || al.bytes == 0) return BEER_EINVAL;
+        char* aw = reinterpret_cast<char*>(prime_acc_ws);
+        prime = {reinterpret_cast<double*>(aw + al.Sp), (size_t)G * af.nslab * 4,
+                 reinterpret_cast<int*>(aw + al.tab), af.nslab};
+    }
     const int Kreal = S * G, nk = nk16_of(cov, D);
     LlhxArgs a = {};
     a.nframes = nframes, a.D = D, a.K = S * f.Gp, a.S = S, a.G = f.Gp;
@@ -1984,11 +2026,13 @@
                                             packed_tiles_bytes(nframes, a.K));
         a.xt_floats = xt_pieces(D) * (kPiece / 4);
     }
-    hipLaunchKernelGGL(const_max_kernel, dim3(1), dim3(256), 0, s, cov, D, Kreal, expT, logw, c0);
+    const bool own_c0 = S == 1 && Kreal <= 256;
+    if (!own_c0)
+        hipLaunchKernelGGL(const_max_kernel, dim3(1), dim3(256), 0, s, cov, D, Kreal, expT, logw, c0);
     hipLaunchKernelGGL(packx_kernel, dim3(f.nchunks * f.NT * 16), dim3(256),
                        (size_t)stats_dim(cov, D) * sizeof(float), s, cov, D, Kreal, f.NT, expT, logw,
                        reinterpret_cast<unsigned short*>(ws), tab, G, f.Gp, c0,
-                       f.lane_major ? 1 : 0);
+                       f.lane_major ? 1 : 0, own_c0 ? 1 : 0, prime);
     BEER_LAUNCH_CHECK();
     const int nku = f.lnfi ? f.nku : 0, gq = f.lnfi ? f.lnfi_g : f.GQ;
     for (const LlhxRow& r : kLlhxRows)
@@ -2095,17 +2139,19 @@
 
 int acc_bf16x3_packed(int cov, int64_t nframes, int D, int K, const float* X, const void* Rimg,
                       double* acc, void* ws, size_t ws_bytes, hipStream_t s, int S, int G,
-                      const float* SR) {
+                      const float* SR, bool primed) {
     const AccxForm f = accx_form(cov, D, K, S, G, SR != nullptr);
     const AccxLayout l = accx_layout(cov, nframes, D, K, S, G, SR != nullptr);
     if (f.rc != BEER_OK || ws_bytes < l.bytes) return BEER_EINVAL;
     char* w = reinterpret_cast<char*>(ws);
     double* Sp = reinterpret_cast<double*>(w + l.Sp);
     int* tab = reinterpret_cast<int*>(w + l.tab);
-    hipError_t e = hipMemsetAsync(Sp, 0, (size_t)K * f.nslab * 4 * sizeof(double), s);
-    if (e != hipSuccess) return -(int)e;
-    hipLaunchKernelGGL(tabx_kernel, dim3(1), dim3(256), 0, s, cov, D, f.nslab, tab);
-    BEER_LAUNCH_CHECK();
+    if (!primed) {
+        hipError_t e = hipMemsetAsync(Sp, 0, (size_t)K * f.nslab * 4 * sizeof(double), s);
+        if (e != hipSuccess) return -(int)e;
+        hipLaunchKernelGGL(tabx_kernel, dim3(1), dim3(256), 0, s, cov, D, f.nslab, tab);
+        BEER_LAUNCH_CHECK();
+    }
     const int64_t tiles = (nframes + kAxFT - 1) / kAxFT;
     const float* Xt;
     if (f.xt_reused) {
@@ -2141,9 +2187,112 @@
     for (const auto& r : kAccxRows)
         if (r.sr == f.sr && r.NQ == f.NQ) {
             const int rc = r.launch(a);
-            return rc != BEER_OK ? rc : unpackx(cov, D, K, Sp, acc, s);
+            return rc != BEER_OK || !acc ? rc : unpackx(cov, D, K, Sp, acc, s);
         }
     return BEER_EINVAL;
+}
+
+
+namespace {
+
+__global__ __launch_bounds__(256) void mixture_tail_kernel(MixtureTail t, int nstat) {
+    __shared__ double red[8];
+    __shared__ unsigned last;
+    const int cov = t.cov, D = t.D, K = t.K, Q = stats_dim(cov, D);
+    const int nq = nslabx_of(cov, D) * 4;
+    const float scale = (float)t.stat_scale;
+    const int bi = blockIdx.x;
+    const int b = bi < t.nutt ? nstat + 1 + bi : (bi == t.nutt ? nstat : bi - t.nutt - 1);
+    auto count = [&](int k) {
+        return 0.0 + -0.5 * t.Sp[(size_t)k * nq + slabx_pos(cov, D, -1, 0)];
+    };
+    if (b < nstat) {
+        const int64_t idx = (int64_t)b * 256 + threadIdx.x;
+        if (idx >= (int64_t)K * Q) return;
+        const int k = (int)(idx / Q), q = (int)(idx % Q);
+        const double* s = t.Sp + (size_t)k * nq;
+        double v;
+        if (q < D) {
+            v = s[slabx_pos(cov, D, q, -1)];
+        } else if (q >= Q - 2) {
+            const double n = s[slabx_pos(cov, D, -1, 0)];
+            v = (q == Q - 2) ? -0.5 * n : (cov == BEER_ISO ? 0.5 * (double)D * n : 0.5 * n);
+        } else if (cov == BEER_FULL) {
+            v = -0.5 * s[slabx_pos(cov, D, (q - D) / D, (q - D) % D)];
+        } else if (cov == BEER_DIAG) {
+            v = -0.5 * s[slabx_pos(cov, D, q - D, q - D)];
+        } else {
+            double tot = 0.0;
+            for (int d = 0; d < D; ++d) tot += s[slabx_pos(cov, D, d, d)];
+            v = -0.5 * tot;
+        }
+        const float f = (float)(0.0 + v);
+        t.stats[idx] = f;
+        t.stats_scaled[idx] = f * scale;
+        return;
+    }
+    if (b == nstat) {
+        if (threadIdx.x >= 64) return;
+        const int lane = threadIdx.x;
+        double tot = 0.0;
+        for (int g = lane; g < K; g += 64) {
+            const double n = -2.0 * count(g);
+            tot += n;
+            if (g < K - 1) {
+                const float f = (float)(0.0 + n);
+                t.wstats[g] = f;
+                t.wstats_scaled[g] = f * scale;
+            }
+        }
+        tot = wave_sum(tot);
+        if (lane == 0) {
+            const float f = (float)(0.0 + tot);
+            t.wstats[K - 1] = f;
+            t.wstats_scaled[K - 1] = f * scale;
+        }
+        return;
+    }
+    const int u = b - nstat - 1;
+    const int64_t f0 = t.frame_off[u], f1 = t.frame_off[u + 1];
+    double sum = 0.0;
+    for (int64_t i = f0 + threadIdx.x; i < f1; i += blockDim.x) sum += (double)t.log_norm[i];
+    sum = block_sum(sum, red);
+    if (threadIdx.x == 0) {
+        const double llh = 0.0 + sum;
+        t.utt_llh[u] = llh;
+        __hip_atomic_store(t.terms + u, t.utt_scale[u] * llh, __ATOMIC_RELAXED,
+                           __HIP_MEMORY_SCOPE_AGENT);
+        asm volatile("s_waitcnt vmcnt(0)" ::: "memory");
+        const unsigned drawn = __hip_atomic_fetch_add(t.ticket, 1u, __ATOMIC_RELAXED,
+                                                      __HIP_MEMORY_SCOPE_AGENT);
+        last = drawn == (unsigned)t.nutt - 1;
+        if (last) {
+            __builtin_amdgcn_fence(__ATOMIC_ACQUIRE, "agent");
+            asm volatile("s_waitcnt vmcnt(0)" ::: "memory");
+        }
+    }
+    __syncthreads();
+    if (!last) return;
+    double v = 0.0;
+    for (int i = threadIdx.x; i < t.nutt; i += blockDim.x)
+        v += __hip_atomic_load(t.terms + i, __ATOMIC_RELAXED, __HIP_MEMORY_SCOPE_AGENT);
+    v = block_sum(v, red);
+    if (threadIdx.x == 0) {
+        t.value[0] = v - (double)t.nutt * (t.kl ? (double)t.kl[0] : 0.0);
+        __hip_atomic_store(t.ticket, 0u, __ATOMIC_RELAXED, __HIP_MEMORY_SCOPE_AGENT);
+    }
+}
+
+}
+
+int mixture_tail(const MixtureTail& t, hipStream_t s) {
+    if (!supported_acc_x(t.D, t.K) || t.nutt < 1) return BEER_EINVAL;
+    const int64_t total = (int64_t)t.K * stats_dim(t.cov, t.D);
+    const int nstat = (int)((total + 255) / 256);
+    hipLaunchKernelGGL(mixture_tail_kernel, dim3((unsigned)(nstat + 1 + t.nutt)), dim3(256), 0, s, t,
+                       nstat);
+    BEER_LAUNCH_CHECK();
+    return BEER_OK;
 }
 
 
@@ -2293,7 +2442,7 @@
     hipLaunchKernelGGL(const_max_kernel, dim3(1), dim3(256), 0, s, cov, D, Kreal, expT, logw, c0);
     hipLaunchKernelGGL(packx_kernel, dim3(kpad), dim3(256),
                        (size_t)stats_dim(cov, D) * sizeof(float), s, cov, D, Kreal, NTC, expT, logw,
-                       reinterpret_cast<unsigned short*>(P), tab, G, f.Gp, c0, 0);
+                       reinterpret_cast<unsigned short*>(P), tab, G, f.Gp, c0, 0, 0, AccPrime{});
     BEER_LAUNCH_CHECK();
     const int waves = f.waves;
     const int rounds = beer::option(BEER_OPT_ACCF_ROUNDS);
diff --git a/beer_amd/csrc/estep_mfma.h b/beer_amd/csrc/estep_mfma.h
--- a/beer_amd/csrc/estep_mfma.h
+++ b/beer_amd/csrc/estep_mfma.h
@@ -30,7 +30,7 @@
 int estep_bf16x3(int cov, int64_t T, int D, int S, int G, const float* X, const float* expT,
                  const float* logw, float* resps, float* log_norm, double* llh_sum, void* ws,
                  size_t ws_bytes, hipStream_t s, bool packed = false,
-                 const void* frame_image = nullptr);
+                 const void* frame_image = nullptr, void* prime_acc_ws = nullptr);
 
 struct LlhForm {
     int NT, GQ, jw, gl, nchunks;
@@ -110,7 +110,22 @@
 size_t accx_workspace_bytes(int cov, int64_t T, int D, int K);
 int acc_bf16x3_packed(int cov, int64_t T, int D, int K, const float* X, const void* Rimg,
                       double* acc, void* ws, size_t ws_bytes, hipStream_t s, int S = 1, int G = 0,
-                      const float* SR = nullptr);
+                      const float* SR = nullptr, bool primed = false);
+struct MixtureTail {
+    int cov, D, K, nutt;
+    const double* Sp;
+    const float* log_norm;
+    const int64_t* frame_off;
+    const double* utt_scale;
+    const float* kl;
+    double stat_scale;
+    float *stats, *stats_scaled;
+    float *wstats, *wstats_scaled;
+    double *utt_llh, *terms;
+    unsigned* ticket;
+    double* value;
+};
+int mixture_tail(const MixtureTail& t, hipStream_t s);
 bool supported_llh_packed_sets(int cov, int D, int S, int G);
 bool supported_acc_sets(int cov, int D, int S, int G);
 size_t accxs_workspace_bytes(int cov, int64_t T, int D, int S, int G);
diff --git a/beer_amd/inference/batch.py b/beer_amd/inference/batch.py
--- a/beer_amd/inference/batch.py
+++ b/beer_amd/inference/batch.py
@@ -10,6 +10,7 @@
 from ..models.modelset import JointModelSet
 from ..models.sequence import HMM, BigramPhoneLoop, PhoneLoop
 from ..models.vae import VAE
+from ..models.weights import Categorical
 from ..stats import FrameStats
 from .objectives import EvidenceLowerBoundInstance
 
@@ -172,15 +173,47 @@
     return t.to(dtype=param.stats.dtype, device=param.stats.device)
 
 
-def _mixture_batch(model, X, lengths, datasize, labels, max_frames, statics=None):
+def _handover_ok(model, X, K, cov, runs, labels, dev):
+    if labels is not None or model.nested or len(runs) != 1 or \
+            not isinstance(model.categorical, Categorical):
+        return False
+    wparam = model.categorical.mean_field_factorization()[0][0]
+    refs = (getattr(wparam, 'stats', None), getattr(model.normalset.means_precisions, 'stats', None))
+    if not all(isinstance(t, torch.Tensor) and t.dtype == torch.float32 and t.device == dev
+               for t in refs):
+        return False
+    return kernels.packed_path_ok(FrameStats(X, cov), K, cov)
+
+
+def _mixture_handover(model, X, lengths, datasize, statics, skey, off_dev, scales, kl, kl_done):
+    ns = model.normalset
+    K, cov = len(ns), ns.cov_type
+    stats = FrameStats(X, cov)
+    done = _throttle()
+    log_norm, resps = kernels.mixture_estep_packed(
+        stats, ns.means_precisions.natural_form(), model._log_weights().view(1, K), K, cov,
+        prime=True)
+    sums = kernels.packed_accumulate_sums(stats, resps, cov)
+    scratch = statics.entry(skey, 'tail_scratch',
+                            lambda: kernels.mixture_tail_scratch(len(lengths), X.device))
+    if kl_done is not None:
+        torch.cuda.current_stream(X.device).wait_event(kl_done)
+    kl_in = kl if isinstance(kl, torch.Tensor) and kl.dtype == torch.float32 and \
+        kl.device == X.device and kl.numel() == 1 and not kl.requires_grad else None
+    st, st_scaled, wst, wst_scaled, _, value = kernels.mixture_tail(
+        sums, log_norm, off_dev, scales, kl_in, datasize / sum(lengths), K, X.shape[1], cov, scratch)
+    done.record()
+    if kl_in is None:
+        value = value - float(len(lengths)) * kl.to(value.device, torch.float64)
+    wparam = model.categorical.mean_field_factorization()[0][0]
+    return value, {wparam: wst, ns.means_precisions: st}, \
+        {wparam: wst_scaled, ns.means_precisions: st_scaled}
+
+
+def _mixture_batch(model, X, lengths, datasize, labels, max_frames, statics=None, kl=None):
     ns = model.normalset
     K, cov = len(ns), ns.cov_type
     dev, dtype = X.device, X.dtype
-    exp_T = ns.means_precisions.natural_form()
-    lw = model._log_weights().view(1, K)
-    Q = FrameStats(X[:1], cov).shape[1]
-    acc = torch.zeros(K, Q, dtype=torch.float64, device=dev)
-    utt_llh = torch.zeros(len(lengths), dtype=torch.float64, device=dev)
 
     def offsets_and_scales():
         off = torch.zeros(len(lengths) + 1, dtype=torch.int64)
@@ -192,12 +225,20 @@
     statics.bind(lengths)
     skey = ('mixture', len(lengths), float(datasize), str(dev))
     off, off_dev, scales = statics.entry(skey, 'offsets', offsets_and_scales)
+    runs = _sub_batches(lengths, K * X.element_size(), max_frames)
+    if kl is not None and _handover_ok(model, X, K, cov, runs, labels, dev):
+        return _mixture_handover(model, X, lengths, datasize, statics, skey, off_dev, scales, *kl)
+    exp_T = ns.means_precisions.natural_form()
+    lw = model._log_weights().view(1, K)
+    Q = FrameStats(X[:1], cov).shape[1]
+    acc = torch.zeros(K, Q, dtype=torch.float64, device=dev)
+    utt_llh = torch.zeros(len(lengths), dtype=torch.float64, device=dev)
     lab_dev = None if labels is None else \
         _hip.on_device(torch.as_tensor(labels)).to(torch.int64).contiguous()
     if lab_dev is not None and model.nested:
         M = len(model.modelset)
         lw_sets = model.modelset.leaf_log_weights()
-    for run in _sub_batches(lengths, K * X.element_size(), max_frames):
+    for run in runs:
         done = _throttle()
         f0, f1 = int(off[run[0]]), int(off[run[-1] + 1])
         stats = FrameStats(X[f0:f1], cov)
@@ -223,7 +264,7 @@
         done.record()
     value_terms = (scales * utt_llh).sum()
     out = {**model._weights_accumulate(acc), ns.means_precisions: _like(ns.means_precisions, acc)}
-    return value_terms, out
+    return value_terms, out, None
 
 
 def _emission_estep(groups, stats, dtype, for_accumulate=False):
@@ -483,7 +524,12 @@
         return EvidenceLowerBoundInstance(0., {}, [], 0, datasize)
     kl, kl_done = _kl_beside_the_estep(model, X.device)
     if isinstance(model, Mixture):
-        value_terms, acc = _mixture_batch(model, X, lengths, datasize, labels, max_frames, statics)
+        value_terms, acc, ready = _mixture_batch(model, X, lengths, datasize, labels, max_frames,
+                                                 statics, kl=(kl, kl_done))
+        if ready is not None:
+            model.clear_cache()
+            return EvidenceLowerBoundInstance(value_terms, acc, model.bayesian_parameters(),
+                                              total, datasize, ready=ready)
     elif isinstance(model, HMM):
         value_terms, acc = _hmm_batch(model, X, lengths, datasize, inference_graphs, scale,
                                       viterbi, state_paths, max_frames, frame_images, statics,
diff --git a/beer_amd/inference/objectives.py b/beer_amd/inference/objectives.py
--- a/beer_amd/inference/objectives.py
+++ b/beer_amd/inference/objectives.py
@@ -22,12 +22,13 @@
 
 class EvidenceLowerBoundInstance:
 
-    def __init__(self, value, acc_stats, model_parameters, minibatchsize, datasize):
+    def __init__(self, value, acc_stats, model_parameters, minibatchsize, datasize, ready=None):
         self.value = value
         self._acc_stats = acc_stats
         self._model_parameters = set(model_parameters)
         self._minibatchsize = minibatchsize
         self._datasize = datasize
+        self._ready = ready
 
     def __repr__(self):
         return f'EvidenceLowerBoundInstance(value={self.value})'
@@ -52,7 +53,11 @@
         if std_params and isinstance(self.value, torch.Tensor) and self.value.requires_grad:
             (-self.value).backward()
         scale = self._datasize / self._minibatchsize
+        ready, self._ready = getattr(self, '_ready', None) or {}, None
         for parameter in self._model_parameters:
+            if parameter in ready:
+                parameter.store_stats(ready[parameter])
+                continue
             try:
                 parameter.store_stats(scale * self._acc_stats[parameter])
             except KeyError:
diff --git a/beer_amd/kernels.py b/beer_amd/kernels.py
--- a/beer_amd/kernels.py
+++ b/beer_amd/kernels.py
@@ -114,7 +114,7 @@
         lib.beer_accumulate_packed_workspace_bytes(code, X.shape[0], D, K) > 0
 
 
-def mixture_estep_packed(stats, exp_stats, log_weights, K, cov_type, llh_sum=None):
+def mixture_estep_packed(stats, exp_stats, log_weights, K, cov_type, llh_sum=None, prime=False):
     st = _frames(stats)
     X = st.data
     T, D = X.shape
@@ -125,12 +125,53 @@
     log_norm = torch.empty(T, 1, dtype=X.dtype, device=X.device)
     words = torch.empty(_hip.lib().beer_packed_resps_bytes(T, D, K) // 4, dtype=torch.int32,
                         device=X.device)
-    ws, ws_bytes = _hip.workspace('beer_estep_workspace_bytes', X.dtype,
-                                  _hip.COV_CODE[cov_type], D, 1, K, X.device)
-    _hip.call('beer_mixture_estep_packed', _hip.COV_CODE[cov_type], T, D, K, _hip.ptr(X),
+    code = _hip.COV_CODE[cov_type]
+    packed = PackedResps(words, T, K)
+    if prime:
+        off = _hip.lib().beer_handover_workspace_offset(code, D, K)
+        acc_bytes = _hip.lib().beer_accumulate_packed_workspace_bytes(code, T, D, K)
+        ws, ws_bytes = _hip.scratch(('handover', code, D, K), off + acc_bytes, X.device)
+        packed.primed = (ws[off:], acc_bytes)
+        code |= _hip.HANDOVER_PRIME
+    else:
+        ws, ws_bytes = _hip.workspace('beer_estep_workspace_bytes', X.dtype, code, D, 1, K, X.device)
+    _hip.call('beer_mixture_estep_packed', code, T, D, K, _hip.ptr(X),
               _hip.ptr(E), _hip.ptr(lw), _hip.ptr(log_norm), _hip.ptr(words), _hip.ptr(llh_sum),
               _hip.ptr(ws), ws_bytes)
-    return log_norm, PackedResps(words, T, K)
+    return log_norm, packed
+
+
+def packed_accumulate_sums(stats, packed, cov_type):
+    X = _frames(stats).data
+    T, D = X.shape
+    ws, ws_bytes = packed.primed
+    if tuple(packed.shape)[0] != T:
+        raise ValueError('packed responsibilities: same frames')
+    _hip.call('beer_normal_accumulate_packed',
+              _hip.COV_CODE[cov_type] | _hip.HANDOVER_PRIMED | _hip.HANDOVER_SUMS, T, D,
+              packed.shape[1], _hip.ptr(X), _hip.ptr(packed.words), None, _hip.ptr(ws), ws_bytes)
+    return ws
+
+
+def mixture_tail(sums, log_norm, frame_off, utt_scale, kl, stat_scale, K, D, cov_type, scratch):
+    dev = log_norm.device
+    n_utts = utt_scale.numel()
+    Q = {'full': D * D + D + 2, 'diagonal': 2 * D + 2, 'isotropic': D + 3}[cov_type]
+    stats = torch.empty(2, K, Q, dtype=torch.float32, device=dev)
+    wstats = torch.empty(2, K, dtype=torch.float32, device=dev)
+    utt_llh = torch.empty(n_utts, dtype=torch.float64, device=dev)
+    value = torch.empty((), dtype=torch.float64, device=dev)
+    _hip.call('beer_mixture_tail', _hip.COV_CODE[cov_type], D, K, n_utts, _hip.ptr(sums),
+              _hip.ptr(log_norm), _hip.ptr(frame_off), _hip.ptr(utt_scale), _hip.ptr(kl),
+              float(stat_scale), _hip.ptr(stats[0]), _hip.ptr(stats[1]), _hip.ptr(wstats[0]),
+              _hip.ptr(wstats[1]), _hip.ptr(utt_llh), _hip.ptr(value), _hip.ptr(scratch),
+              scratch.numel())
+    return stats[0], stats[1], wstats[0], wstats[1], utt_llh, value
+
+
+def mixture_tail_scratch(n_utts, device):
+    return torch.zeros(_hip.lib().beer_mixture_tail_scratch_bytes(n_utts), dtype=torch.uint8,
+                       device=device)
 
 
 def packed_sets_ok(stats, S, G, cov_type):
diff --git a/include/beer_hip.h b/include/beer_hip.h
--- a/include/beer_hip.h
+++ b/include/beer_hip.h
@@ -146,6 +146,16 @@
                                   const void* packed_resps, double* acc,
                                   void* workspace, size_t workspace_bytes,
                                   void* stream);
+#define BEER_HANDOVER_PRIME 0x100
+#define BEER_HANDOVER_PRIMED 0x100
+#define BEER_HANDOVER_SUMS 0x200
+size_t beer_handover_workspace_offset(int cov, int D, int K);
+size_t beer_mixture_tail_scratch_bytes(int32_t n_utts);
+int beer_mixture_tail(int cov, int D, int K, int32_t n_utts, const void* sums,
+                      const float* log_norm, const int64_t* frame_off, const double* utt_scale,
+                      const float* kl, double stat_scale, float* stats, float* stats_scaled,
+                      float* weight_stats, float* weight_stats_scaled, double* utt_llh,
+                      double* value, void* scratch, size_t scratch_bytes, void* stream);
 int beer_mixtureset_packed_supported(int cov, int D, int S, int G);
 size_t beer_mixtureset_accumulate_packed_workspace_bytes(int cov, int64_t T, int D, int S,
                                                          int G);
```

Measured after the change: 271.5 million (median of 2 runs). About the same (+0.7%).
